# dsilvestro/LiteRate

Measured on AMD Instinct MI355X. Metric: RJMCMC iters/sec x lineages (lineage-log-lik evals/s, summed over chains), higher is better.
Workload: dtype f64

## Files before the change

include/literate_hip.h:

```cpp
#ifndef LITERATE_HIP_H
#define LITERATE_HIP_H

#include <stdint.h>

#ifdef __cplusplus
extern "C" {
#endif

#define LR_OK 0
#define LR_ERR_NULL (-1)
#define LR_ERR_SIZE (-2)
#define LR_ERR_MODEL (-3)
#define LR_ERR_WORKSPACE (-4)
#define LR_ERR_T0 (-5)
#define LR_ERR_STATE (-6)
#define LR_ERR_ORDER (-7)

#define LR_KMAX 32
#define LR_ROW 64
#define LR_MAX_BINS 4094

#define LR_MODEL_BD 0
#define LR_MODEL_ID 1
#define LR_MODEL_KEIDING 2
// ... 177 lines not shown
    int32_t persistent;
    int32_t reserved1;
    int64_t status;
    int64_t xchg;
    int32_t team_blocks;
    int32_t table_mode;
    int64_t lineage_frac;
    int64_t pack_tmp;
    int32_t spec_chains_per_team;
    int32_t streaming;
    int32_t packed_scan;
    int32_t reserved3;
} lr_mcmc_layout;

#define LR_ROW_L 0
#define LR_ROW_M 1
#define LR_ROW_TL 2
#define LR_ROW_TM 3
#define LR_ROW_PL 4
#define LR_ROW_PM 5
#define LR_ROW_PTL 6
#define LR_ROW_PTM 7
#define LR_ROW_SCALARS 8
#define LR_STATE_ROWS 9
#define LR_S_LIKA 0
#define LR_S_PRIORA 1
#define LR_S_PRIORPOIA 2
#define LR_S_GRATE_L 3
#define LR_S_GRATE_M 4
#define LR_S_POI 5
#define LR_S_HASTING 6
#define LR_S_PRIOR_P 7
#define LR_S_PRIORPOI_P 8
#define LR_S_CONST_P 9
#define LR_S_CONST_A 10
#define LR_S_LIK_P 11
#define LR_S_LOG_G0 12
#define LR_S_LOG_G1 13
#define LR_S_LOG_POI 14
#define LR_S_LOG_U 15
#define LR_IROW_EL 0
#define LR_IROW_EM 1
#define LR_IROW_PEL 2
#define LR_IROW_PEM 3
#define LR_IROW_SCALARS 4
#define LR_ISTATE_ROWS 5
#define LR_I_KL 0
#define LR_I_KM 1
#define LR_I_PKL 2
#define LR_I_PKM 3
#define LR_I_GIBBS 4
#define LR_I_INVALID 5
#define LR_I_IT_LO 6
#define LR_I_IT_HI 7
#define LR_I_ACCEPTED 8
#define LR_I_MOVE 9
#define LR_I_NEXT_LO 10
#define LR_I_NEXT_HI 11
#define LR_I_SLOT 12

#define LR_TRACE_HEAD 13
#define LR_TRACE_W (LR_TRACE_HEAD + 2 * (2 * LR_KMAX - 1))

typedef struct lr_engine lr_engine;

int lr_mcmc_query_layout(const lr_mcmc_config* cfg , lr_mcmc_layout* out );
int lr_mcmc_create(const lr_mcmc_config* cfg , const double* ts, const double* te,
                   const double* br_length ,
                   void* workspace, int64_t workspace_bytes, lr_engine** out );
int lr_mcmc_init(lr_engine* e, const double* L, const double* M, const double* tL,
                 const double* tM, const int32_t* KL, const int32_t* KM, int32_t kmax, void* stream);
int lr_mcmc_steps(lr_engine* e, int64_t n_iters, void* stream);
int lr_mcmc_restore(lr_engine* e, void* stream);
int lr_mcmc_time_scan(lr_engine* e, int32_t reps, float* avg_ms , void* stream);
int lr_mcmc_time_steps(lr_engine* e, int64_t n_iters, float* total_ms , void* stream);
int lr_mcmc_status(lr_engine* e, int32_t* status , void* stream);
#define LR_WARN_KCAP 2
int lr_mcmc_warnings(lr_engine* e, int32_t* warnings , void* stream);
int lr_mcmc_describe(const lr_engine* e, char* buf , int32_t n);
int lr_mcmc_p4_config(const lr_engine* e, int32_t* word );
int lr_mcmc_p4_resident(const lr_engine* e, int32_t out[4] );
int lr_mcmc_p4_pipe(const lr_engine* e, int32_t out[4] );
int lr_mcmc_p4_draws(const lr_engine* e, int32_t* out );
int lr_mcmc_destroy(lr_engine* e);

#ifdef __cplusplus
}
#endif
#endif
```

literate_amd/_hip.py:

```python
import ctypes as C
import os

from .build import LIB

c_i32, c_i64, c_f64, c_vp = C.c_int32, C.c_int64, C.c_double, C.c_void_p

LR_ERR_NULL, LR_ERR_SIZE, LR_ERR_MODEL, LR_ERR_WORKSPACE, LR_ERR_T0, LR_ERR_STATE, LR_ERR_ORDER = -1, -2, -3, -4, -5, -6, -7
ERRORS = {-1: "LR_ERR_NULL", -2: "LR_ERR_SIZE", -3: "LR_ERR_MODEL", -4: "LR_ERR_WORKSPACE", -5: "LR_ERR_T0",
          -6: "LR_ERR_STATE", -7: "LR_ERR_ORDER (lineages must be sorted by birth time for the persistent engines)"}

LR_KMAX, LR_ROW, LR_MAX_BINS = 32, 64, 4094
LR_ADE_MAX_BINS = 512
LR_ADEJ_MAX_BINS, LR_ADEJ_MOVES, LR_ADEJ_STATE_W, LR_ADEJ_ROW_W = 128, 5, 96, 73
LR_MLIK_MAX_BINS, LR_MLIK_MAX_TEMPS, LR_MLIK_MOVES, LR_MLIK_STATE_W, LR_MLIK_ROW_W = 512, 128, 2, 16, 12
LR_TMLIK_MAX_BINS, LR_TMLIK_MAX_TEMPS, LR_TMLIK_MAX_MODELS, LR_TMLIK_MOVES, LR_TMLIK_STATE_W, LR_TMLIK_ROW_W = 512, 128, 64, 2, 16, 12
LR_RJBIN_MAX_BINS, LR_RJBIN_STATE_W = 512, 448
LR_RJMC3_MAX_TEMPS, LR_RJMC3_S_POS, LR_RJMC3_LADDER_W, LR_RJMC3_WIDE_MAX_BINS, LR_P_SWAP = 8, 9, 4, 256, 11
LR_WARN_KCAP = 2
LR_STATE_ROWS, LR_ISTATE_ROWS = 9, 5
LR_TRACE_HEAD = 13
LR_TRACE_W = LR_TRACE_HEAD + 2 * (2 * LR_KMAX - 1)
LR_SIMBATCH_GROUPS, LR_SIMBATCH_LDS_SLOTS = 512, 16384
LR_SHIFT_PRIOR_KCAP, LR_SHIFT_PRIOR_BLOCKS = 64, 768
LR_ESS_LDS_ROWS = 16384
# ... 45 lines not shown

SIGNATURES = {
    "lr_version": (c_i32, []),
    "lr_bin_events_workspace_bytes": (c_i64, [c_i64, c_i32]),
    "lr_bin_events": (c_i32, [c_vp, c_vp, c_i64, c_vp, c_vp, c_i32, c_vp, c_vp, c_vp, c_vp, c_i64, c_vp]),
    "lr_bin_unit_events_workspace_bytes": (c_i64, [c_i64, c_i32]),
    "lr_bin_unit_events": (c_i32, [c_vp, c_vp, c_i64, c_f64, c_i32, c_vp, c_vp, c_vp, c_vp, c_i64, c_vp]),
    "lr_expand_rates": (c_i32, [c_vp, c_vp, c_vp, c_i32, c_i32, c_i32, c_i32, c_vp, c_vp]),
    "lr_bd_loglik_workspace_bytes": (c_i64, [c_i64, c_i32, c_i32, c_i32]),
    "lr_bd_loglik_plan": (c_i32, [c_i64, c_i32, c_i32, c_i32, C.POINTER(c_i32)]),
    "lr_bd_loglik_batch": (c_i32, [c_vp, c_vp, c_i64, c_f64, c_i32, c_vp, c_vp, c_i32, c_i32, c_vp, c_f64, c_vp,
                                   c_vp, c_i64, c_vp]),
    "lr_waic_workspace_bytes": (c_i64, [c_i64, c_i32, c_i32, c_i32]),
    "lr_waic_plan": (c_i32, [c_i64, c_i32, c_i32, c_i32, C.POINTER(c_i32)]),
    "lr_waic_pointwise": (c_i32, [c_vp, c_vp, c_i64, c_f64, c_i32, c_vp, c_vp, c_i32, c_i32, c_vp, c_f64, c_vp, c_vp, c_vp,
                                  c_i64, c_vp]),
    "lr_loo_workspace_bytes": (c_i64, [c_i64, c_i32, c_i32, c_i32]),
    "lr_loo_plan": (c_i32, [c_i64, c_i32, c_i32, c_i32, C.POINTER(c_i32)]),
    "lr_loo_pointwise": (c_i32, [c_vp, c_vp, c_i64, c_f64, c_i32, c_vp, c_vp, c_i32, c_i32, c_vp, c_f64, c_vp, c_vp, c_vp,
                                 c_i64, c_vp]),
    "lr_psis_rows_workspace_bytes": (c_i64, [c_i64, c_i32]),
    "lr_psis_rows": (c_i32, [c_vp, c_i64, c_i32, c_vp, c_vp, c_vp, c_i64, c_vp]),
    "lr_rj_propose_score": (c_i32, [c_vp, c_vp, c_vp, c_i32, c_i32, c_vp, c_vp, c_vp, c_f64, c_vp, c_vp, c_vp, c_vp,
                                    c_vp]),
    "lr_log_priors": (c_i32, [c_vp, c_vp, c_i32, c_i32, c_f64, c_vp, c_vp, c_vp, c_vp]),
    "lr_dd_rates": (c_i32, [c_vp, c_vp, c_i32, c_i32, c_i32, c_i32, c_vp, c_vp, c_vp, c_vp, c_vp]),
    "lr_ddv2_rates": (c_i32, [c_vp, c_vp, c_i32, c_i32, c_i32, c_i32, c_vp, c_vp, c_vp, c_vp, c_vp]),
    "lr_binned_keiding": (c_i32, [c_vp, c_vp, c_vp, c_vp, c_vp, c_i32, c_i32, c_vp, c_vp, c_vp]),
    "lr_simulate_bd": (c_i32, [c_vp, c_vp, c_i32, c_i32, c_f64, c_f64, c_f64, c_f64, c_i64, c_i64, C.c_uint64, c_vp, c_vp,
                             c_vp, c_vp, c_vp, c_i64, c_vp]),
    "lr_simulate_bd_batch_workspace_bytes": (c_i64, [c_i32, c_i32, c_i32, c_i64]),
    "lr_simulate_bd_batch": (c_i32, [c_vp, c_vp, c_i32, c_i32, c_i32, c_vp, c_i64, C.c_uint64, c_vp, c_vp, c_vp, c_i64,
                                   c_vp]),
    "lr_simulate_dd_batch_workspace_bytes": (c_i64, [c_i32, c_i32, c_i32, c_i64]),
    "lr_simulate_dd_batch": (c_i32, [c_vp, c_vp, c_i32, c_i32, c_i32, c_i32, c_i32, c_vp, c_i64, C.c_uint64, c_vp, c_vp, c_vp,
                                   c_i64, c_vp]),
    "lr_trend_rates": (c_i32, [c_vp, c_vp, c_i32, c_i32, c_i32, c_i32, c_vp, c_vp, c_vp]),
    "lr_format_rows": (c_i64, [c_vp, c_vp, c_i64, C.c_uint64, c_i32, c_vp, c_i64]),
    "lr_rtt_summary_workspace_bytes": (c_i64, [c_i32, c_i32, c_f64, c_f64, c_f64, c_i32]),
    "lr_rtt_summary": (c_i32, [c_vp, c_i32, c_i32, c_f64, c_f64, c_f64, c_i32, c_vp, c_vp, c_vp, c_vp, c_i64, c_vp]),
    "lr_shift_prior": (c_i32, [c_f64, c_f64, c_i64, c_i64, C.c_uint64, c_f64, c_i32, c_vp, c_vp, c_vp, c_vp, c_vp]),
    "lr_ppc_age_workspace_bytes": (c_i64, [c_i64, c_i32, c_i32]),
    "lr_ppc_age_plan": (c_i32, [c_i64, c_i32, c_i32, C.POINTER(c_i32)]),
    "lr_ppc_age": (c_i32, [c_vp, c_vp, c_i64, c_f64, c_i32, c_vp, c_i32, C.c_uint64, c_vp, c_vp, c_vp, c_vp, c_i64, c_vp]),
    "lr_ade_classes": (c_i32, [c_vp, c_vp, c_i64, c_f64, c_i32, c_vp, c_vp, c_vp, c_vp]),
    "lr_ade_profile_workspace_bytes": (c_i64, [c_i32, c_i32, c_i32]),
    "lr_ade_profile": (c_i32, [c_vp, c_vp, c_i32, c_vp, c_i32, c_vp, c_i32, c_vp, c_vp, c_vp, c_vp, c_i64, c_vp]),
    "lr_adej_workspace_bytes": (c_i64, [c_i32]),
    "lr_adej_prepare": (c_i32, [c_vp, c_vp, c_i32, c_vp, c_i64, c_vp]),
    "lr_adej_loglik": (c_i32, [c_vp, c_i64, c_i32, c_vp, c_vp, c_i32, c_vp, c_vp, c_vp]),
    "lr_adej_init": (c_i32, [c_vp, c_i64, c_i32, c_f64, c_i32, c_i32, c_f64, c_f64, C.c_uint64, c_i32, c_i32, c_vp, c_vp]),
    "lr_adej_steps": (c_i32, [c_vp, c_i64, c_i32, c_f64, c_i32, c_i32, c_f64, c_f64, C.c_uint64, c_i32, c_i32, c_vp, c_i64, c_i64,
                              c_i32, c_vp, c_i64, c_vp]),
    "lr_mlik_init": (c_i32, [c_vp, c_vp, c_vp, c_i32, c_f64, c_f64, c_i32, c_i32, c_f64, c_vp, c_vp, c_i32, C.c_uint64, c_i32, c_i32,
                             c_vp, c_vp]),
    "lr_mlik_steps": (c_i32, [c_vp, c_vp, c_vp, c_i32, c_f64, c_f64, c_i32, c_i32, c_f64, c_vp, c_vp, c_i32, C.c_uint64, c_i32, c_i32,
                              c_vp, c_i64, c_i64, c_i32, c_vp, c_i64, c_vp]),
    "lr_mlik_estimate": (c_i32, [c_vp, c_i64, c_i32, c_i32, c_i64, c_vp, c_vp, c_vp, c_vp, c_vp, c_vp, c_vp, c_vp]),
    "lr_tmlik_init": (c_i32, [C.POINTER(TmlikProblem)]),
    "lr_tmlik_steps": (c_i32, [C.POINTER(TmlikProblem), c_i64, c_i64, c_i32, c_vp, c_i64, c_i64]),
    "lr_rjbin_init": (c_i32, [C.POINTER(RjbinProblem), c_vp, c_vp, c_vp, c_vp, c_vp, c_vp]),
    "lr_rjbin_steps": (c_i32, [C.POINTER(RjbinProblem), c_i64, c_i64, c_i32, c_vp, c_i64, c_i64]),
    "lr_rjmc3_init": (c_i32, [C.POINTER(Rjmc3Problem), c_vp, c_vp, c_vp, c_vp, c_vp, c_vp]),
    "lr_rjmc3_steps": (c_i32, [C.POINTER(Rjmc3Problem), c_i64, c_i64, c_i32, c_vp, c_vp, c_i64, c_i64]),
    "lr_ess_summary_workspace_bytes": (c_i64, [c_i32, c_i32, c_i32, c_vp, c_i32, c_f64, c_i32]),
    "lr_ess_summary": (c_i32, [c_vp, c_i32, c_i32, c_i32, c_vp, c_i32, c_f64, c_i32, c_vp, c_vp, c_vp, c_vp, c_i64, c_vp]),
    "lr_col_summary_workspace_bytes": (c_i64, [c_i32, c_i32, c_i32, c_vp, c_i32, c_f64, c_i32, c_i32]),
    "lr_col_summary": (c_i32, [c_vp, c_i32, c_i32, c_i32, c_vp, c_i32, c_f64, c_i32, c_vp, c_vp, c_i64, c_vp]),
    "lr_curve_summary_workspace_bytes": (c_i64, [c_i32, c_i32, c_i32, c_i32, c_i32, c_i32, c_f64, c_i32, c_i32]),
    "lr_curve_summary": (c_i32, [c_vp, c_i32, c_i32, c_i32, c_i32, c_i32, c_i32, c_i32, c_vp, c_i32, c_f64, c_i32, c_vp,
                                 c_vp, c_i64, c_vp]),
    "lr_mcmc_query_layout": (c_i32, [C.POINTER(McmcConfig), C.POINTER(McmcLayout)]),
    "lr_mcmc_create": (c_i32, [C.POINTER(McmcConfig), c_vp, c_vp, c_vp, c_vp, c_i64, C.POINTER(c_vp)]),
    "lr_mcmc_init": (c_i32, [c_vp, c_vp, c_vp, c_vp, c_vp, c_vp, c_vp, c_i32, c_vp]),
    "lr_mcmc_steps": (c_i32, [c_vp, c_i64, c_vp]),
    "lr_mcmc_time_scan": (c_i32, [c_vp, c_i32, C.POINTER(C.c_float), c_vp]),
    "lr_mcmc_time_steps": (c_i32, [c_vp, c_i64, C.POINTER(C.c_float), c_vp]),
    "lr_mcmc_restore": (c_i32, [c_vp, c_vp]),
    "lr_mcmc_describe": (c_i32, [c_vp, C.c_char_p, c_i32]),
    "lr_mcmc_p4_config": (c_i32, [c_vp, C.POINTER(c_i32)]),
    "lr_mcmc_p4_resident": (c_i32, [c_vp, C.POINTER(c_i32)]),
    "lr_mcmc_p4_pipe": (c_i32, [c_vp, C.POINTER(c_i32)]),
    "lr_mcmc_p4_draws": (c_i32, [c_vp, C.POINTER(c_i32)]),
    "lr_mcmc_status": (c_i32, [c_vp, C.POINTER(c_i32), c_vp]),
    "lr_mcmc_warnings": (c_i32, [c_vp, C.POINTER(c_i32), c_vp]),
    "lr_mcmc_destroy": (c_i32, [c_vp]),
    "lr_debug_draws": (c_i32, [C.c_uint64, c_i64, c_vp, c_vp, c_vp, c_vp, c_vp, c_i32, c_vp, c_vp]),
    "lr_debug_stream2": (c_i32, [c_vp, c_vp, c_i64, c_vp, c_vp]),
}

_lib = None


class HipLibraryError(RuntimeError):
    pass


def load():
    global _lib
    if _lib is not None:
        return _lib
    if not os.path.exists(LIB):
        raise HipLibraryError("libliterate_hip.so not found at %s - run `python -m literate_amd.build` "
                              "(there is no CPU fallback)" % LIB)
    lib = C.CDLL(LIB)
    for name, (res, args) in SIGNATURES.items():
        fn = getattr(lib, name)
        fn.restype, fn.argtypes = res, args
    _lib = lib
    return lib


def check(rc, what):
    if rc == 0:
        return
    if rc < 0:
        raise ValueError("%s: %s" % (what, ERRORS.get(rc, rc)))
    raise HipLibraryError("%s: hipError_t %d" % (what, rc))


def require_gpu():
    import torch
    if not torch.cuda.is_available():
        raise HipLibraryError("no ROCm GPU visible: literate_amd has no CPU path")
    return torch


def ptr(t):
    return None if t is None else c_vp(t.data_ptr())


def stream_ptr(device=None):
    import torch
    return c_vp(torch.cuda.current_stream(device).cuda_stream)


def launch(fn, device, *args):
    import torch
    with torch.cuda.device(device):
        return fn(*args, stream_ptr(device))


def launch_problem(fn, device, problem, *args):
    import torch
    with torch.cuda.device(device):
        problem.stream = stream_ptr(device)
        return fn(C.byref(problem), *args)
```

literate_amd/csrc/lr_engine.h:

```cpp
#pragma once
#include <cmath>
#include "lr_internal.h"
#include "lr_plan.h"
#include "lr_scan.h"
#include "lr_step.h"

struct lr_part {
    int base, count, hA;
    bool pipelined;
    hipStream_t stream;
    hipEvent_t done;
    hipGraphExec_t graph_exec;
    int graph_units;
};

struct lr_p4_shares {
    int delta[16];
    int n_slots;
    int help_trips;
};

struct lr_engine {
    lr_mcmc_config cfg;
    lr_mcmc_layout lay;
    lr_engine_plan plan;
    const double* ts;
    const double* te;
    const double* br_length;
    char* ws;
    bool initialised;
    lr_part part[LR_MAX_PARTS];
    long long n8;
    long long n8_alloc;
    lr_p4_shares p4;
    bool p4_help;
    int p4_cfg;
    bool p4_resident;
    bool p4_pipe;
    bool p4_lean;
    bool packed_scan;
    bool streaming;
    hipEvent_t fork;
    hipEvent_t ev0, ev1;
};


#ifndef LR_SPEC_SCAN_UNROLL
#define LR_SPEC_SCAN_UNROLL 1
#endif
#ifndef LR_SPEC_SCAN_PRIO
#define LR_SPEC_SCAN_PRIO 2
#endif
#define LR_SPEC_TIMEOUT_TICKS 200000000ull

static inline bool lr_p4_help_choice(const lr_engine* e) {
    const char* env = getenv("LR_P4_HELP");
    if (e->lay.persistent != 2 || e->plan.scan.unit == LR_TAB_PAIRGEN || e->cfg.sampler != 0 || e->plan.scan.H > 264) return false;
    return env ? atoi(env) != 0 : true;
}

static inline int lr_p4_cfg_choice(const lr_engine* e) {
    const char* env = getenv("LR_P4_GENERIC");
    if (!lr_p4_help_choice(e) || (env && atoi(env) != 0)) return LR_P4_CFG_GENERIC;
    const lr_mcmc_config& c = e->cfg;
    if (c.const_rates != 0 || c.use_rate_HP == 0 || c.poisson_HP != 0.0) return LR_P4_CFG_GENERIC;
    if (c.frac_birth != LR_P4_FRAC_BIRTH || std::signbit(c.frac_birth) || c.frac_death != LR_P4_FRAC_DEATH) return LR_P4_CFG_GENERIC;
    if (c.model == LR_MODEL_BD || c.model == LR_MODEL_ID) return LR_P4_CFG_BDI;
    return c.model == LR_MODEL_KEIDING ? LR_P4_CFG_KEIDING : LR_P4_CFG_GENERIC;
}

static inline bool lr_p4_resident_choice(const lr_engine* e) {
    const char* env = getenv("LR_P4_RESIDENT");
    return lr_p4_help_choice(e) && !(env && atoi(env) == 0);
}

static inline bool lr_p4_pipe_choice(const lr_engine* e) {
    const char* env = getenv("LR_P4_PIPE");
    return lr_p4_resident_choice(e) && !(env && atoi(env) == 0);
}

static inline bool lr_p4_lean_choice(const lr_engine* e) {
    const char* env = getenv("LR_P4_LEAN_DRAWS");
    return lr_p4_pipe_choice(e) && !(env && atoi(env) == 0);
}

static inline int lr_spec_mode(const lr_engine* e) {
    if (e->lay.spec_chains_per_team != 1) return 0;
    if (e->lay.team_blocks > 1) return 1;
    const double trips = (double)e->n8 / 64.0 / 8.0;
    const char* env = getenv("LR_SPEC_PLANES_BY_SCANNERS");
    const bool by_scanners = env ? atoi(env) != 0 : trips <= 3.0;
    return by_scanners ? 2 : 3;
}

#define LR_STEP_WAVES_PER_BLOCK (LR_SCAN_THREADS / LR_WAVE)
#define LR_STREAM_MAX_CHAINS 16
struct lr_stream_sync {
    unsigned long long arrived;
    unsigned long long pad0[15];
    unsigned long long word[LR_STREAM_COPIES][LR_STREAM_MAX_CHAINS];
};
static_assert(sizeof(lr_stream_sync) + 128 == LR_STREAM_SYNC_BYTES && LR_STREAM_SYNC_BYTES % 256 == 0, "counter line + a line per copy");
int lr_launch_stream(lr_engine* e, const lr_step_args& a, int64_t n_iters, bool query, hipStream_t stream);

int lr_packscan_pairs(const lr_scan_plan& p, int n_chains);
int lr_launch_packscan(const lr_engine* e, int base, int count, hipStream_t stream);

lr_step_args lr_make_args(const lr_engine* e);
int lr_pack_lineages(lr_engine* e, hipStream_t stream);
int lr_launch_spec(lr_engine* e, const lr_step_args& a, const lr_packed_lineages& pk, int64_t n_iters, hipStream_t stream);
```

literate_amd/csrc/lr_mcmc.hip:

```cpp
#include <cmath>
#include <cstdio>
#include <cstdlib>
#include <new>
#include <type_traits>

#include "lr_chain.h"
#include "lr_dd.h"
#include "lr_engine.h"
#include "lr_internal.h"
#include "lr_scan.h"
#include "lr_step.h"

__global__ __launch_bounds__(LR_WAVE) void lr_rj_propose_score_kernel(
    const double* __restrict__ rates, const double* __restrict__ times, const int* __restrict__ K, int kmax,
    const int* __restrict__ move, const int* __restrict__ index, const double* __restrict__ draws, double mult_d,
    double* __restrict__ out_rates, double* __restrict__ out_times, int* __restrict__ out_K,
    double* __restrict__ out_score) {
    const int c = blockIdx.x, lane = threadIdx.x;
    int k = K[c];
    double R = (lane < k) ? rates[(size_t)c * kmax + lane] : 0.0;
    double T = (lane <= k) ? times[(size_t)c * (kmax + 1) + lane] : 0.0;
    const double* dr = draws + (size_t)c * 2 * kmax;
    const int mv = move[c];
    double score = 0.0;
// ... 74 lines not shown

__global__ __launch_bounds__(LR_SCAN_THREADS) void lr_chain_step_kernel(lr_step_args a, int mode, int chain_base,
                                                                        int n_sub) {
    __shared__ lr_seg_scratch scratch[LR_STEP_WAVES];
    const int wave = threadIdx.x / LR_WAVE, lane = threadIdx.x & (LR_WAVE - 1);
    const int j = blockIdx.x * LR_STEP_WAVES + wave;
    if (j < n_sub) lr_chain_step_body<32>(a, mode, chain_base + j, lane, &scratch[wave]);
}

struct lr_fused_args {
    const double* ts;
    const double* te;
    long long n, chunk;
    double t0;
    int n_bins, tiles;
    int scan_base, scan_n;
    int step_base, step_n;
    int step_blocks;
};

template <int CB, int H, bool UNIT>
__global__ __launch_bounds__(LR_SCAN_THREADS) void lr_fused_iter_kernel(lr_step_args a, lr_fused_args f) {
    extern __shared__ double2 lds[];
    lr_seg_scratch* scratch = reinterpret_cast<lr_seg_scratch*>(lds);
    const int bid = blockIdx.x;
    if (bid < f.step_blocks) {
        const int wave = threadIdx.x / LR_WAVE, lane = threadIdx.x & (LR_WAVE - 1);
        const int j = bid * LR_STEP_WAVES + wave;
        if (j < f.step_n) lr_chain_step_body(a, 0, f.step_base + j, lane, &scratch[wave]);
        return;
    }
    int group, tile;
    if ((f.step_blocks & 7) == 0) {
        lr_xcd_remap(bid - f.step_blocks, f.tiles, (f.scan_n + CB - 1) / CB, &group, &tile);
    } else {
        const int sb = bid - f.step_blocks;
        tile = sb % f.tiles, group = sb / f.tiles;
    }
    const double2* tables = a.tables + (size_t)f.scan_base * a.tab_stride;
    const int tile_stride = lr_tile_stride(a.tiles);
    double* partials = const_cast<double*>(a.partials) + (size_t)f.scan_base * tile_stride;
    if (UNIT)
        lr_scan_unit_body<CB, H>(lds, tile, group * CB, f.ts, f.te, f.n, f.t0, f.n_bins, tables, f.scan_n, f.chunk,
                                 partials, tile_stride);
    else
        lr_scan_fast_body<CB, H>(lds, tile, group * CB, f.ts, f.te, f.n, f.t0, f.n_bins, tables, f.scan_n, f.chunk,
                                 partials, tile_stride);
}

#ifndef LR_PERSIST_THREADS
#define LR_PERSIST_THREADS 512
#endif
#ifndef LR_PERSIST_MINWAVES
#define LR_PERSIST_MINWAVES 4
#endif

template <int H, bool GENERAL>
__global__ __launch_bounds__(256) void lr_pairscan_kernel(lr_packed_lineages pk, long long n8, const double2* __restrict__ tables,
                                                          int n_chains, int n_bins, int tiles, double* __restrict__ partials) {
    constexpr int ENT = GENERAL ? 2 : 1;
    __shared__ double2 tab[LR_UNIT_PLANES * H];
    __shared__ double red[4][2];
    const int tid = threadIdx.x, lane = tid & (LR_WAVE - 1), wave = tid / LR_WAVE;
    const int tile = blockIdx.x, pair = blockIdx.y;
    const double2* src = tables + (size_t)pair * (2 * H * ENT);
    for (int i = tid; i < 2 * H * ENT; i += 256) tab[GENERAL ? lr_pairgen_lds_entry(i, H) : i] = src[i];
    __syncthreads();
    if (GENERAL) lr_pair_planes_block_general(tab, H, n_bins, tid, 256);
    else lr_pair_planes_block(tab, H, n_bins, tid, 256);
    __syncthreads();
    const long long per = (n8 + tiles - 1) / tiles;
    const long long g0 = min((long long)tile * per, n8), g1 = min(g0 + per, n8);
    double acc0 = 0.0, acc1 = 0.0;
    lr_persist_scan<H, GENERAL>(reinterpret_cast<const char*>(tab), pk, g0, g1 - g0, tid, 256, &acc0, &acc1);
    const double s0 = lr_wave_sum(acc0), s1 = lr_wave_sum(acc1);
    if (lane == 0) red[wave][0] = s0, red[wave][1] = s1;
    __syncthreads();
    if (tid < 2 && 2 * pair + tid < n_chains)
        partials[(size_t)(2 * pair + tid) * lr_tile_stride(tiles) + tile] = ((red[0][tid] + red[1][tid]) + red[2][tid]) + red[3][tid];
}

typedef __attribute__((address_space(3))) double lr_lds_f64;
typedef __attribute__((address_space(3))) int lr_lds_i32;
template <int PB, int ES, bool PRE = false, int SAMPLER = -1, bool HAND = false, int CFG = LR_P4_CFG_GENERIC, bool LEAN = false>
__device__ __forceinline__ void lr_persist_step_body(const __attribute__((address_space(3))) lr_step_args* a3, int c, int lane,
                                                     __attribute__((address_space(3))) lr_seg_scratch* scratch3,
                                                     lr_lds_f64* st_f64, lr_lds_i32* st_i32, double lik, lr_lds_f64* table3,
                                                     lr_lds_f64* br3 ,
                                                     const lr_draw_slot* draws = nullptr ,
                                                     lr_table_hand* hand = nullptr, int hand_epoch = 0) {
    constexpr int table_es = ES;
    const lr_step_args& a = *(const lr_step_args*)a3;
    const double* br_lds = (const double*)br3;
    LR_SSTAMP(0);
    lr_chain_regs st;
    lr_chain_load(st, (double*)st_f64, (int*)st_i32, lane);
    if (SAMPLER == 1 || (SAMPLER == -1 && a.cfg.sampler != 0))
        lr_dd_step_core<true>(st, a, 0, c, lane, lik, reinterpret_cast<double2*>((double*)table3), table_es, br_lds);
    else if (PRE) {
        lr_rj_draws pre;
        lr_draws_load(draws, pre, lane);
        lr_chain_step_core<true, PB, HAND, CFG, LEAN>(st, a, 0, c, lane, (lr_seg_scratch*)scratch3, lik, reinterpret_cast<double2*>((double*)table3),
                                           table_es, br_lds, br_lds + LR_H_WIDE, &pre, hand, hand_epoch);
    } else
        lr_chain_step_core<true, PB>(st, a, 0, c, lane, (lr_seg_scratch*)scratch3, lik, reinterpret_cast<double2*>((double*)table3),
                                     table_es, br_lds, br_lds + LR_H_WIDE);
    if (HAND) lr_chain_store_handed(st, (double*)st_f64, (int*)st_i32, lane);
    else lr_chain_store(st, (double*)st_f64, (int*)st_i32, lane);
    LR_SSTAMP(8);
}

template <int NA, int BATCH = NA>
__device__ __forceinline__ void lr_p4_leave_sums(double2 (*part)[LR_WAVE], int* arrived, double* out, int slot, int lane,
                                                 int& scans_done, double s0, double s1) {
    part[slot][lane] = make_double2(s0, s1);
    int prev = 0;
    if (lane == 0) prev = __hip_atomic_fetch_add(arrived, 1, __ATOMIC_RELAXED, __HIP_MEMORY_SCOPE_WORKGROUP);
    prev = __builtin_amdgcn_readfirstlane(prev);
    if (prev == NA * (scans_done + 1) - 1) {
        asm volatile("" ::: "memory");
        double a0 = 0.0, a1 = 0.0;
#pragma unroll
        for (int w = 0; w < NA; ++w) {
            if (BATCH < NA && w > 0 && w % BATCH == 0) asm volatile("" : "+v"(a0), "+v"(a1) :: "memory");
            const double2 v = part[w][lane];
            a0 += v.x, a1 += v.y;
        }
        a0 = lr_wave_sum(a0), a1 = lr_wave_sum(a1);
        if (lane == 0) out[0] = a0, out[1] = a1;
    }
    ++scans_done;
}

template <int PB, int ES>
__device__ __attribute__((noinline)) void lr_persist_step(const __attribute__((address_space(3))) lr_step_args* a3, int c, int lane,
                                                          __attribute__((address_space(3))) lr_seg_scratch* scratch3,
                                                          lr_lds_f64* st_f64, lr_lds_i32* st_i32, double lik, lr_lds_f64* table3,
                                                          lr_lds_f64* br3) {
    lr_persist_step_body<PB, ES>(a3, c, lane, scratch3, st_f64, st_i32, lik, table3, br3);
}

template <int PB, int ES, int NW, int SAMPLER, bool HELP, int CFG = LR_P4_CFG_GENERIC, int TAG = 0, bool LEAN = false>
__device__ __attribute__((noinline)) void lr_persist4_steppers(const __attribute__((address_space(3))) lr_step_args* a3, int c0,
                                                               int n_chains, int wave, int lane,
                                                               __attribute__((address_space(3))) lr_seg_scratch* scratch3,
                                                               lr_lds_f64* st_f64, lr_lds_i32* st_i32, lr_lds_f64* red,
                                                               lr_lds_f64* tab, int tab_doubles, lr_lds_f64* br3, long long n_iters,
                                                               const lr_draw_slot* draws ,
                                                               lr_table_hand* hands ) {
    static_assert(!HELP || (ES == 2 && SAMPLER == 0), "helper waves: RJ sampler at unit resolution");
    static_assert(CFG == LR_P4_CFG_GENERIC || HELP, "a configuration word comes with the helper waves");
    for (long long iter = 0; iter < n_iters; ++iter) {
#pragma unroll 1
        for (int ph = 0; ph < 2; ++ph) {
#ifdef LR_DIAG
            const unsigned long long dq0 = wall_clock64();
#endif
            const int c = c0 + 2 * ph + wave;
            if (c < n_chains) {
                double lik = 0.0;
#pragma unroll
                for (int w2 = 2; w2 < (ES == 2  ? 3 : NW); ++w2) lik += red[(ph * NW + w2) * 2 + wave];
                lr_persist_step_body<PB, ES, ES == 2  && SAMPLER == 0, SAMPLER, HELP, CFG, LEAN>(
                    a3, c, lane, scratch3, st_f64 + (2 * ph + wave) * (LR_STATE_ROWS * LR_ROW),
                    st_i32 + (2 * ph + wave) * (LR_ISTATE_ROWS * LR_ROW), lik, tab + ph * tab_doubles + wave, br3,
                    draws + (2 * ph + wave), HELP ? hands + wave : nullptr, (int)((2 * iter + ph + 1) & 0x3fffffff));
            }
#ifdef LR_DIAG
            const unsigned long long dq1 = wall_clock64();
#endif
            __syncthreads();
#ifdef LR_DIAG
            if (lane == 0 && blockIdx.x < 64) {
                atomicAdd(&lr_diag_step[16384 + (blockIdx.x * 16 + wave) * 4 + 0], dq1 - dq0);
                atomicAdd(&lr_diag_step[16384 + (blockIdx.x * 16 + wave) * 4 + 1], wall_clock64() - dq1);
            }
#endif
        }
    }
}

template <int H, int T, int PB>
__device__ __attribute__((noinline)) void lr_persist2_steppers(const __attribute__((address_space(3))) lr_step_args* a3, int c, int wave,
                                                               int lane, __attribute__((address_space(3))) lr_seg_scratch* scratch3,
                                                               lr_lds_f64* st_f64, lr_lds_i32* st_i32, lr_lds_f64* red ,
                                                               lr_lds_f64* tab, lr_lds_f64* br3, const uint4* __restrict__ idx8,
                                                               long long n8w, long long n_iters, int prio_shift, int grp) {
    const int tid = wave * LR_WAVE + lane;
    for (long long iter = 0; iter < n_iters; ++iter) {
        if (prio_shift > 0) {
            if (((wall_clock64() >> prio_shift) + grp) & 1) __builtin_amdgcn_s_setprio(1);
            else __builtin_amdgcn_s_setprio(0);
        }
        double acc0 = 0.0, acc1 = 0.0;
        lr_scan_tail tail;
        lr_persist_scan_pair<H, 1, true>((const char*)(const double*)tab, idx8, n8w, tid, T, &acc0, &acc1, nullptr, &tail);
        const double s0 = lr_wave_sum(acc0), s1 = lr_wave_sum(acc1);
        if (lane == 0) red[wave * 2 + 0] = s0, red[wave * 2 + 1] = s1;
        lr_scan_drain(tail);
        __syncthreads();
        double lik = 0.0;
#pragma unroll
        for (int w2 = 0; w2 < T / LR_WAVE; ++w2) lik += red[w2 * 2 + wave];
        lr_persist_step_body<PB, 2>(a3, c, lane, scratch3, st_f64, st_i32, lik, tab + wave, br3);
        __syncthreads();
    }
}

template <int H, int T>
__global__ __launch_bounds__(T, LR_PERSIST_MINWAVES) void lr_persist_kernel(
    const lr_step_args* __restrict__ ap ,
    const uint4* __restrict__ idx8, long long n8, lr_p4_shares sh, long long n_iters, int prio_shift) {
    const lr_step_args& a = *ap;
    __shared__ double2 tab[LR_UNIT_PLANES * H];
    __shared__ double red[T / LR_WAVE][2];
    __shared__ lr_seg_scratch scratch[2];
    __shared__ double st_f64[2][LR_STATE_ROWS * LR_ROW];
    __shared__ int st_i32[2][LR_ISTATE_ROWS * LR_ROW];
    __shared__ lr_step_args a_lds;
    __shared__ double br_lds[2][LR_H_WIDE];
    const int tid = threadIdx.x, lane = tid & (LR_WAVE - 1), wave = tid / LR_WAVE;
    if (tid < (int)(sizeof(lr_step_args) / 4)) reinterpret_cast<int*>(&a_lds)[tid] = reinterpret_cast<const int*>(ap)[tid];
    for (int b = tid; b < LR_H_WIDE; b += blockDim.x) {
        const bool in = b < ap->cfg.n_bins;
        br_lds[0][b] = (in && ap->br_length) ? ap->br_length[b] : 0.0;
        br_lds[1][b] = in ? ap->log_br[b] : 0.0;
    }
    const int c0 = blockIdx.x * 2;
    const int c = c0 + wave;
    const bool stepper = (wave < 2) && (c < a.cfg.n_chains);
    double2* gpair = lr_chain_table(a, c0);
    if (stepper) {
        const double* S = a.state_f64 + (size_t)c * LR_STATE_ROWS * LR_ROW;
        const int* I = a.state_i32 + (size_t)c * LR_ISTATE_ROWS * LR_ROW;
        for (int r = 0; r < LR_STATE_ROWS; ++r) st_f64[wave][r * LR_ROW + lane] = S[r * LR_ROW + lane];
        for (int r = 0; r < LR_ISTATE_ROWS; ++r) st_i32[wave][r * LR_ROW + lane] = I[r * LR_ROW + lane];
    }
    for (int i = tid; i < 2 * H; i += T) tab[i] = gpair[i];
    __syncthreads();
    lr_pair_planes_block(tab, H, a.cfg.n_bins, tid, T);
    __syncthreads();
    const char* lbase = reinterpret_cast<const char*>(tab);
    const long long n8w = sh.delta[0] != 0 ? ((n8 + T - 1) / T + sh.delta[wave]) * T : n8;
    const int grp = (blockIdx.x >> 8) & 1;
#ifdef LR_DIAG
    unsigned long long d_t0 = 0, d_t1 = 0, d_t2 = 0, d_scan = 0, d_red = 0, d_step = 0;
// ... 8 lines not shown
    } else
#endif
    for (long long iter = 0; iter < n_iters; ++iter) {
        if (prio_shift > 0) {
            if (((wall_clock64() >> prio_shift) + grp) & 1) __builtin_amdgcn_s_setprio(1);
            else __builtin_amdgcn_s_setprio(0);
        }
#ifdef LR_DIAG
        d_t0 = wall_clock64();
#endif
        double acc0 = 0.0, acc1 = 0.0;
        lr_scan_tail tail;
        lr_persist_scan_pair<H, 1, true>(lbase, idx8, n8w, tid, T, &acc0, &acc1, nullptr, &tail);
#ifdef LR_DIAG
        if (lane == 0 && blockIdx.x < 512) atomicAdd(&lr_diag_step[20000 + blockIdx.x * 8 + wave], wall_clock64() - d_t0);
#endif
#ifdef LR_DIAG
        d_t1 = wall_clock64();
#endif
        const double s0 = lr_wave_sum(acc0), s1 = lr_wave_sum(acc1);
        if (lane == 0) red[wave][0] = s0, red[wave][1] = s1;
        lr_scan_drain(tail);
        __syncthreads();
#ifdef LR_DIAG
        d_t2 = wall_clock64();
#endif
        if (stepper) {
            double lik = 0.0;
#pragma unroll
            for (int w2 = 0; w2 < T / LR_WAVE; ++w2) lik += red[w2][wave];
            lr_persist_step<(H <= 264 ? lr_bins_per_lane(H) : 0), 2>(
                (const __attribute__((address_space(3))) lr_step_args*)&a_lds, c, lane,
                (__attribute__((address_space(3))) lr_seg_scratch*)&scratch[wave], (lr_lds_f64*)st_f64[wave],
                (lr_lds_i32*)st_i32[wave], lik, (lr_lds_f64*)(reinterpret_cast<double*>(tab) + wave), (lr_lds_f64*)&br_lds[0][0]);
        }
        __syncthreads();
#ifdef LR_DIAG
        d_scan += d_t1 - d_t0, d_red += d_t2 - d_t1, d_step += wall_clock64() - d_t2;
#endif
    }
#ifdef LR_DIAG
    if (lane == 0 && blockIdx.x < 512) {
        unsigned long long* o = lr_diag_step + 4096 * 12 - 4096 + (blockIdx.x * 8 + wave) % 4096;
        (void)o;
    }
    if (tid == 0 && blockIdx.x < 340) {
        lr_diag_step[blockIdx.x * 12 + 9] = d_scan, lr_diag_step[blockIdx.x * 12 + 10] = d_red;
        lr_diag_step[blockIdx.x * 12 + 11] = d_step;
    }
    if (tid == 0 && blockIdx.x < 1024) lr_diag_step[2048 * 12 + blockIdx.x * 2 + 1] = wall_clock64();
#endif
    if (stepper) {
        double* S = a.state_f64 + (size_t)c * LR_STATE_ROWS * LR_ROW;
        int* I = a.state_i32 + (size_t)c * LR_ISTATE_ROWS * LR_ROW;
        for (int r = 0; r < LR_STATE_ROWS; ++r) S[r * LR_ROW + lane] = st_f64[wave][r * LR_ROW + lane];
        for (int r = 0; r < LR_ISTATE_ROWS; ++r) I[r * LR_ROW + lane] = st_i32[wave][r * LR_ROW + lane];
    }
    for (int i = tid; i < 2 * H; i += T) gpair[i] = tab[i];
}

#ifndef LR_P4_THREADS
#define LR_P4_THREADS 1024
#endif
#ifdef LR_DIAG
#define LR_PSTAMP(k) if (threadIdx.x == 0 && blockIdx.x < 64) lr_diag_step[28672 + blockIdx.x * 8 + (k)] = wall_clock64()
#else
#define LR_PSTAMP(k)
#endif

#ifndef LR_P4_NR
#define LR_P4_NR 8
#endif
#ifndef LR_P4_RES_HDR
#define LR_P4_RES_HDR 0
#endif
#ifndef LR_P4_NR_DRAW
#define LR_P4_NR_DRAW 4
#endif
#define LR_P4_RES_HELP 5
#ifndef LR_P4_PIPE
#define LR_P4_PIPE 1
#endif
template <int H, bool GENERAL, bool PARAM ,
          bool HELP = false, int CFG = LR_P4_CFG_GENERIC, int NR = 0, int PIPE = 0, bool LEAN = false>
__global__ __launch_bounds__(LR_P4_THREADS, LR_P4_THREADS / 256) void lr_persist4_kernel(const lr_step_args* __restrict__ ap ,
                                                                       lr_packed_lineages pk, long long n8,
                                                                       lr_p4_shares sh, long long n_iters, char* carry_all) {
    static_assert(!HELP || (!GENERAL && !PARAM), "helper waves: RJ sampler at unit resolution");
    static_assert(CFG == LR_P4_CFG_GENERIC || (HELP && H <= 264), "a configuration word comes with the helper waves");
    static_assert(NR == 0 || HELP, "resident groups come with the helper waves");
    static_assert(PIPE == 0 || (PIPE == 1 && NR > 0), "the one-block form is one of the resident trips");
    static_assert(!LEAN || PIPE > 0, "the lean draw duty comes with the one-block form");
    const lr_step_args& a = *ap;
    LR_PSTAMP(0);
    constexpr int NW = LR_P4_THREADS / LR_WAVE;
    constexpr int W0 = HELP ? 4 : 2;
    constexpr int NS = NW - W0;
    constexpr int LR_P4_SCANNERS = NS * LR_WAVE;
    constexpr int ENT = GENERAL ? 2 : 1;
    constexpr int ES = GENERAL ? 6 * H : 2;
    __shared__ double2 tab[2][LR_UNIT_PLANES * H];
    __shared__ double red[2][NW][2];
    constexpr bool LAST_SUMS = !GENERAL;
    __shared__ double2 part[LAST_SUMS ? NW - 2 : 1][LR_WAVE];
    __shared__ int arrived;
    __shared__ lr_table_hand hands[2];
    __shared__ lr_seg_scratch scratch[2];
    __shared__ double st_f64[4][LR_STATE_ROWS * LR_ROW];
    __shared__ int st_i32[4][LR_ISTATE_ROWS * LR_ROW];
    __shared__ lr_step_args a_lds;
    __shared__ double br_lds[2][LR_H_WIDE];
    __shared__ lr_draw_slot draws_s[4];
    lr_draw_slot* const draws = draws_s;
    const int tid = threadIdx.x, lane = tid & (LR_WAVE - 1), wave = tid / LR_WAVE;
    if (tid < (int)(sizeof(lr_step_args) / 4)) reinterpret_cast<int*>(&a_lds)[tid] = reinterpret_cast<const int*>(ap)[tid];
    for (int b = tid; b < LR_H_WIDE; b += blockDim.x) {
        const bool in = b < ap->cfg.n_bins;
        br_lds[0][b] = (in && ap->br_length) ? ap->br_length[b] : 0.0;
        br_lds[1][b] = in ? ap->log_br[b] : 0.0;
    }
    constexpr bool draw_ahead = !GENERAL && !PARAM;
    auto draw_duty = [&](int pr) {
        const int q = wave - W0, k = q & 1, ch = 2 * pr + k;
        if (!draw_ahead || q < 0 || q >= (HELP ? 2 : 4) || (int)(blockIdx.x * 4) + ch >= ap->cfg.n_chains) return;
        const int* I = st_i32[ch] + LR_IROW_SCALARS * LR_ROW;
        const unsigned long long it = ((unsigned long long)(unsigned int)I[LR_I_IT_HI] << 32 | (unsigned int)I[LR_I_IT_LO]) + 1ull;
        lr_draw_slot* slot = &draws[ch];
        if (LEAN) lr_spec_draw_lean<CFG>(a_lds, (int)(blockIdx.x * 4) + ch, lane, it, slot, I);
        else if (HELP) lr_spec_draw_both<CFG>(a_lds, (int)(blockIdx.x * 4) + ch, lane, it, slot);
        else lr_spec_draw_part(a_lds, (int)(blockIdx.x * 4) + ch, lane, it, slot, q >> 1);
    };
    auto help_duty = [&](int ph, int epoch) {
        const int k = wave - 2;
        const int ch = 2 * ph + k;
        if ((int)(blockIdx.x * 4) + ch >= ap->cfg.n_chains) return;
        lr_table_hand* hand = &hands[k];
#ifdef LR_DIAG
        const unsigned long long dh0 = wall_clock64();
#endif
        while (__hip_atomic_load(&hand->epoch, __ATOMIC_RELAXED, __HIP_MEMORY_SCOPE_WORKGROUP) != epoch) __builtin_amdgcn_s_sleep(1);
        asm volatile("" ::: "memory");
#ifdef LR_DIAG
        if (lane == 0 && blockIdx.x < 64) atomicAdd(&lr_diag_step[16384 + (blockIdx.x * 16 + wave) * 4 + 2], wall_clock64() - dh0);
#endif
        const lr_seg_scratch* sc = &scratch[k];
        const int eL = lane <= LR_KMAX ? sc->edge[0][lane] : 0, eM = lane <= LR_KMAX ? sc->edge[1][lane] : 0;
        double* tabd = reinterpret_cast<double*>(tab[ph]) + k;
        int model = a_lds.cfg.model;
        if (CFG == LR_P4_CFG_BDI) __builtin_assume((unsigned int)model < 2u);
        if (CFG == LR_P4_CFG_KEIDING) model = LR_MODEL_KEIDING;
        constexpr bool fixed = CFG != LR_P4_CFG_GENERIC;
        const double constP = lr_build_tables_segments<(H <= 264 ? lr_bins_per_lane(H) : 1), 2>(
            sc, eL, eM, hand->KL, hand->KM, br_lds[0], br_lds[1], model, a_lds.cfg.n_bins, a_lds.n_cls, fixed ? H : a_lds.H,
            reinterpret_cast<double2*>(tabd), lane, LR_TAB_UNIT, fixed ? LR_P4_FRAC_BIRTH : a_lds.cfg.frac_birth,
            fixed ? LR_P4_FRAC_DEATH : a_lds.cfg.frac_death, ES, nullptr);
        LR_WAVE_LDS_ORDER();
        lr_pair_planes_wave(tabd, H, a_lds.cfg.n_bins, lane, 0);
        if (lane == 0) st_f64[ch][LR_ROW_SCALARS * LR_ROW + LR_S_CONST_P] = constP;
    };
    if (tid == 0) arrived = 0;
    if (tid < 2) hands[tid].epoch = 0;
    for (int i = tid; i < 2 * NW * 2; i += LR_P4_THREADS) (&red[0][0][0])[i] = 0.0;
    int scans_done = 0;
    constexpr int NA = NS + (HELP ? 2 : 0);
    auto leave_sums = [&](int pr, double s0, double s1) {
        if (LAST_SUMS) {
            lr_p4_leave_sums<NA, (NR > 0 ? NA / 2 : NA)>(part, &arrived, &red[pr][2][0], wave >= W0 ? wave - W0 : NS + wave - 2, lane, scans_done, s0, s1);
        } else {
            s0 = lr_wave_sum(s0), s1 = lr_wave_sum(s1);
            if (lane == 0) red[pr][wave][0] = s0, red[pr][wave][1] = s1;
        }
    };
    const int c0 = blockIdx.x * 4;
    const int C = a.cfg.n_chains;
    if (wave < 4 && c0 + wave < C) {
        const int c = c0 + wave;
        const double* S = a.state_f64 + (size_t)c * LR_STATE_ROWS * LR_ROW;
        const int* I = a.state_i32 + (size_t)c * LR_ISTATE_ROWS * LR_ROW;
        for (int r = 0; r < LR_STATE_ROWS; ++r) st_f64[wave][r * LR_ROW + lane] = S[r * LR_ROW + lane];
        for (int r = 0; r < LR_ISTATE_ROWS; ++r) st_i32[wave][r * LR_ROW + lane] = I[r * LR_ROW + lane];
    }
    double2* g0 = lr_chain_table(a, c0);
    double2* g1 = lr_chain_table(a, c0 + 2);
    for (int i = tid; i < 2 * H * ENT; i += LR_P4_THREADS) {
        const int e = GENERAL ? lr_pairgen_lds_entry(i, H) : i;
        tab[0][e] = g0[i], tab[1][e] = g1[i];
    }
    __syncthreads();
    LR_PSTAMP(1);
    if (GENERAL) {
        lr_pair_planes_block_general(tab[0], H, a.cfg.n_bins, tid, LR_P4_THREADS);
        lr_pair_planes_block_general(tab[1], H, a.cfg.n_bins, tid, LR_P4_THREADS);
    } else {
        lr_pair_planes_block(tab[0], H, a.cfg.n_bins, tid, LR_P4_THREADS);
        lr_pair_planes_block(tab[1], H, a.cfg.n_bins, tid, LR_P4_THREADS);
    }
    __syncthreads();
    LR_PSTAMP(2);
    const bool scanner = wave >= W0;
    const bool helper = HELP && (wave == 2 || wave == 3);
    const int sid = tid - W0 * LR_WAVE;
    const long long nh_ = HELP ? (long long)sh.help_trips * (2 * LR_WAVE) : 0;
    const int k_tot = (int)((n8 - nh_ + LR_P4_SCANNERS - 1) / LR_P4_SCANNERS);
    const int k_mine = k_tot + (scanner ? sh.delta[wave - W0] : 0);
    bool any_shift = false;
#pragma unroll
    for (int q = 0; q < NS; ++q) any_shift |= sh.delta[q] != 0;
    const long long nh = HELP ? (long long)sh.help_trips * (2 * LR_WAVE) : 0;
    const long long n8w = any_shift ? (long long)k_mine * LR_P4_SCANNERS : n8 - nh;
    constexpr bool HDR = LR_P4_RES_HDR != 0;
    lr_resident_groups<(NR > 0 ? NR : 1), HDR> res;
    lr_resident_groups<LR_P4_RES_HELP, HDR> hres;
    constexpr int NRD = NR > 0 ? LR_P4_NR_DRAW : 0;
    lr_resident_groups<(NRD > 0 ? NRD : 1), HDR> dres;
    const bool res_scanner = NR > 0 && scanner && !(draw_ahead && wave - W0 < 2);
    auto help_scan = [&](auto pr_, auto resident_) {
        constexpr int pr = decltype(pr_)::value;
        double s0 = 0.0, s1 = 0.0;
        if (decltype(resident_)::value) {
            const long long done = (long long)hres.trips * (2 * LR_WAVE);
            lr_resident_trips<LR_P4_RES_HELP, HDR, (PIPE > 0)>(reinterpret_cast<const char*>(tab[pr]), hres, s0, s1);
            if (nh > done) lr_persist_scan<H, GENERAL, 1, false, false>(reinterpret_cast<const char*>(tab[pr]), pk, done, nh - done, tid - 2 * LR_WAVE, 2 * LR_WAVE, &s0, &s1);
        } else if (nh > 0) lr_persist_scan<H, GENERAL, 1, false, false>(reinterpret_cast<const char*>(tab[pr]), pk, 0, nh, tid - 2 * LR_WAVE, 2 * LR_WAVE, &s0, &s1);
        leave_sums(pr, s0, s1);
    };
    auto scan_resident = [&](auto pr_, double* s0, double* s1, lr_scan_tail* tail) {
        constexpr int pr = decltype(pr_)::value;
        lr_persist_scan_pair_resident<(PIPE > 0)>(reinterpret_cast<const char*>(tab[pr]), pk.idx8 + nh, n8w, sid, LR_P4_SCANNERS, res, s0, s1, tail);
    };
    static_assert(2 * NW * 8 + 4 <= LR_P4_CARRY_BYTES, "");
    char* carry = carry_all ? carry_all + (size_t)blockIdx.x * LR_P4_CARRY_BYTES : nullptr;
    const bool carried = carry && *reinterpret_cast<const int*>(carry + 2 * NW * 8) == 1;
    auto prologue_draws = [&]() { draw_duty(0); };
    if (carried) {
        if (tid < 2 * NW) (&red[0][0][0])[tid] = reinterpret_cast<const double*>(carry)[tid];
        if (scanner) prologue_draws();
    } else if (scanner) {
        double s0 = 0.0, s1 = 0.0;
        lr_scan_tail tail;
        lr_persist_scan<H, GENERAL, 1, false, true>(reinterpret_cast<const char*>(tab[0]), pk, nh, n8w, sid, LR_P4_SCANNERS, &s0, &s1, nullptr, &tail);
        leave_sums(0, s0, s1);
        lr_scan_drain(tail);
        prologue_draws();
    }
    if (helper && !carried) help_scan(std::integral_constant<int, 0>(), std::false_type());
    __syncthreads();
    LR_PSTAMP(3);
    if (helper) {
        if (NR > 0) lr_resident_load(hres, pk.idx8, nh, tid - 2 * LR_WAVE, 2 * LR_WAVE);
        for (long long iter = 0; iter < n_iters; ++iter) {
#pragma unroll 1
            for (int ph = 0; ph < 2; ++ph) {
#ifdef LR_DIAG
                const unsigned long long dq0 = wall_clock64();
#endif
                if (ph == 0) help_scan(std::integral_constant<int, 1>(), std::integral_constant<bool, (NR > 0)>());
                else help_scan(std::integral_constant<int, 0>(), std::integral_constant<bool, (NR > 0)>());
                help_duty(ph, (int)((2 * iter + ph + 1) & 0x3fffffff));
#ifdef LR_DIAG
                const unsigned long long dq1 = wall_clock64();
#endif
                __syncthreads();
#ifdef LR_DIAG
                if (lane == 0 && blockIdx.x < 64) {
                    atomicAdd(&lr_diag_step[16384 + (blockIdx.x * 16 + wave) * 4 + 0], dq1 - dq0);
                    atomicAdd(&lr_diag_step[16384 + (blockIdx.x * 16 + wave) * 4 + 1], wall_clock64() - dq1);
                }
#endif
            }
        }
    } else if (!scanner)
        lr_persist4_steppers<(H <= 264 ? lr_bins_per_lane(H) : 0), ES, NW, PARAM ? 1 : 0, HELP, CFG, NR + 64 * PIPE, LEAN>(
            (const __attribute__((address_space(3))) lr_step_args*)&a_lds, c0, C, wave, lane,
            (__attribute__((address_space(3))) lr_seg_scratch*)&scratch[wave], (lr_lds_f64*)&st_f64[0][0], (lr_lds_i32*)&st_i32[0][0],
            (lr_lds_f64*)&red[0][0][0], (lr_lds_f64*)reinterpret_cast<double*>(tab[0]), 2 * LR_UNIT_PLANES * H,
            (lr_lds_f64*)&br_lds[0][0], n_iters, &draws[0], &hands[0]);
    else if (res_scanner) {
        if constexpr (NR > 0) {
        lr_resident_load(res, pk.idx8 + nh, n8w, sid, LR_P4_SCANNERS);
        for (long long iter = 0; iter < n_iters; ++iter) {
#pragma unroll
            for (int ph = 0; ph < 2; ++ph) {
#ifdef LR_DIAG
                const unsigned long long dq0 = wall_clock64();
#endif
                {
                    double s0 = 0.0, s1 = 0.0;
                    lr_scan_tail tail;
                    if (ph == 0) scan_resident(std::integral_constant<int, 1>(), &s0, &s1, &tail);
                    else scan_resident(std::integral_constant<int, 0>(), &s0, &s1, &tail);
                    leave_sums(1 - ph, s0, s1);
                    lr_scan_drain(tail);
                }
#ifdef LR_DIAG
                const unsigned long long dq1 = wall_clock64();
#endif
                __syncthreads();
#ifdef LR_DIAG
                if (lane == 0 && blockIdx.x < 64) {
                    atomicAdd(&lr_diag_step[16384 + (blockIdx.x * 16 + wave) * 4 + 0], dq1 - dq0);
                    atomicAdd(&lr_diag_step[16384 + (blockIdx.x * 16 + wave) * 4 + 1], wall_clock64() - dq1);
                }
#endif
            }
        }
        }
    } else {
    if constexpr (NRD > 0) lr_resident_load(dres, pk.idx8 + nh, n8w, sid, LR_P4_SCANNERS);
    for (long long iter = 0; iter < n_iters; ++iter) {
#pragma unroll
        for (int ph = 0; ph < 2; ++ph) {
#ifdef LR_DIAG
            const unsigned long long dq0 = wall_clock64();
#endif
            {
                double s0 = 0.0, s1 = 0.0;
                lr_scan_tail tail;
                if constexpr (NRD > 0) {
                    if (ph == 0) lr_persist_scan_pair_resident<(PIPE > 0)>(reinterpret_cast<const char*>(tab[1]), pk.idx8 + nh, n8w, sid, LR_P4_SCANNERS, dres, &s0, &s1, &tail);
                    else lr_persist_scan_pair_resident<(PIPE > 0)>(reinterpret_cast<const char*>(tab[0]), pk.idx8 + nh, n8w, sid, LR_P4_SCANNERS, dres, &s0, &s1, &tail);
                } else
                lr_persist_scan<H, GENERAL, 1, false, true>(reinterpret_cast<const char*>(tab[1 - ph]), pk, nh, n8w, sid, LR_P4_SCANNERS, &s0, &s1, nullptr, &tail);
                leave_sums(1 - ph, s0, s1);
                lr_scan_drain(tail);
                draw_duty(1 - ph);
            }
#ifdef LR_DIAG
            const unsigned long long dq1 = wall_clock64();
#endif
            __syncthreads();
#ifdef LR_DIAG
            if (lane == 0 && blockIdx.x < 64) {
                atomicAdd(&lr_diag_step[16384 + (blockIdx.x * 16 + wave) * 4 + 0], dq1 - dq0);
                atomicAdd(&lr_diag_step[16384 + (blockIdx.x * 16 + wave) * 4 + 1], wall_clock64() - dq1);
            }
#endif
        }
    }
    }
    LR_PSTAMP(4);
    if (wave < 4 && c0 + wave < C) {
        const int c = c0 + wave;
        double* S = a.state_f64 + (size_t)c * LR_STATE_ROWS * LR_ROW;
        int* I = a.state_i32 + (size_t)c * LR_ISTATE_ROWS * LR_ROW;
        for (int r = 0; r < LR_STATE_ROWS; ++r) S[r * LR_ROW + lane] = st_f64[wave][r * LR_ROW + lane];
        for (int r = 0; r < LR_ISTATE_ROWS; ++r) I[r * LR_ROW + lane] = st_i32[wave][r * LR_ROW + lane];
    }
    for (int i = tid; i < 2 * H * ENT; i += LR_P4_THREADS) {
        const int e = GENERAL ? lr_pairgen_lds_entry(i, H) : i;
        g0[i] = tab[0][e], g1[i] = tab[1][e];
    }
    if (carry) {
        if (tid < 2 * NW) reinterpret_cast<double*>(carry)[tid] = (&red[0][0][0])[tid];
        if (tid == 0) *reinterpret_cast<int*>(carry + 2 * NW * 8) = 1;
    }
// ... 40 lines not shown
        } else {
            const lr_dd_params pp = lr_dd_unpack(A);
            lr_dd_build_tables_wave(pp, a.br_length, cfg.m_birth, cfg.m_death, n_bins, a.H, lr_chain_table(a, c), lane,
                                    a.unit, cfg.frac_birth, cfg.frac_death, lr_tab_es(a.unit, a.H));
        }
        for (int r = 0; r < LR_STATE_ROWS; ++r) S[r * LR_ROW + lane] = 0.0;
        for (int r = 0; r < LR_ISTATE_ROWS; ++r) I[r * LR_ROW + lane] = 0;
        S[LR_ROW_L * LR_ROW + lane] = A, S[LR_ROW_PL * LR_ROW + lane] = A;
        int io = 0;
        if (lane == LR_I_KL || lane == LR_I_PKL || lane == LR_I_KM || lane == LR_I_PKM) io = npar;
        I[LR_IROW_SCALARS * LR_ROW + lane] = io;
        return;
    }
    double L = 0.0, M = 0.0, tL = 0.0, tM = 0.0;
    int KL = 1, KM = 1;
    if (L0) {
        KL = KL0[c], KM = KM0[c];
        if (lane < KL) L = L0[(size_t)c * kmax + lane];
        if (lane < KM) M = M0[(size_t)c * kmax + lane];
        if (lane <= KL) tL = tL0[(size_t)c * (kmax + 1) + lane];
        if (lane <= KM) tM = tM0[(size_t)c * (kmax + 1) + lane];
    } else {
        const double l0 = lr_gamma(rng, 0, LR_P_INIT, 0, 2.0) * 2.0;
        const double m0 = lr_gamma(rng, 0, LR_P_INIT, 64, 2.0) * 2.0;
        if (lane == 0) L = l0, M = m0, tL = tM = cfg.start_time;
        if (lane == 1) tL = tM = cfg.end_time;
    }
    const int eL = lr_wave_edges(tL, 1), eM = lr_wave_edges(tM, 1);
    double logL, logM;
    lr_stage_segments(&scratch, L, M, eL, eM, KL, KM, lane, &logL, &logM);
    const double constA = lr_build_tables_segments(&scratch, eL, eM, KL, KM, a.br_length, a.log_br, cfg.model, n_bins,
                                                   a.n_cls, a.H, lr_chain_table(a, c), lane,
                                                   a.unit, cfg.frac_birth, cfg.frac_death, lr_tab_es(a.unit, a.H));
    S[LR_ROW_L * LR_ROW + lane] = L, S[LR_ROW_M * LR_ROW + lane] = M;
    S[LR_ROW_TL * LR_ROW + lane] = tL, S[LR_ROW_TM * LR_ROW + lane] = tM;
    S[LR_ROW_PL * LR_ROW + lane] = L, S[LR_ROW_PM * LR_ROW + lane] = M;
    S[LR_ROW_PTL * LR_ROW + lane] = tL, S[LR_ROW_PTM * LR_ROW + lane] = tM;
    I[LR_IROW_EL * LR_ROW + lane] = eL, I[LR_IROW_EM * LR_ROW + lane] = eM;
    I[LR_IROW_PEL * LR_ROW + lane] = eL, I[LR_IROW_PEM * LR_ROW + lane] = eM;
    const double poi0 = (cfg.poisson_HP == 0.0) ? 1.0 : cfg.poisson_HP;
    double so = 0.0;
    if (lane == LR_S_GRATE_L || lane == LR_S_GRATE_M) so = 1.0;
    if (lane == LR_S_POI) so = poi0;
    if (lane == LR_S_LOG_POI) so = lr_log(poi0);
    if (lane == LR_S_CONST_A || lane == LR_S_CONST_P) so = constA;
    S[LR_ROW_SCALARS * LR_ROW + lane] = so;
    int io = 0;
    if (lane == LR_I_KL || lane == LR_I_PKL) io = KL;
    if (lane == LR_I_KM || lane == LR_I_PKM) io = KM;
    I[LR_IROW_SCALARS * LR_ROW + lane] = io;
}

extern "C" int lr_mcmc_query_layout(const lr_mcmc_config* cfg, lr_mcmc_layout* out) {
    lr_engine_plan plan;
    return lr_plan_layout(cfg, &plan, out);
}

extern "C" int lr_mcmc_create(const lr_mcmc_config* cfg, const double* ts, const double* te, const double* br_length,
                              void* workspace, int64_t workspace_bytes, lr_engine** out) {
    if (!ts || !te || !workspace || !out) return LR_ERR_NULL;
    lr_engine_plan plan;
    lr_mcmc_layout lay;
    int rc = lr_plan_layout(cfg, &plan, &lay);
    if (rc) return rc;
    if ((cfg->model == LR_MODEL_BD || cfg->model == LR_MODEL_ID || cfg->sampler != 0) && !br_length) return LR_ERR_MODEL;
    if (lay.total_bytes > workspace_bytes) return LR_ERR_WORKSPACE;
    lr_engine* e = new (std::nothrow) lr_engine();
    if (!e) return (int)hipErrorOutOfMemory;
    e->cfg = *cfg;
    e->lay = lay;
    e->plan = plan;
    e->ts = ts, e->te = te, e->br_length = br_length;
    e->ws = (char*)workspace;
    e->initialised = false;
    e->n8 = 0;
    e->n8_alloc = lr_groups_alloc(cfg->n_lineages);
    for (int j = 0; j < 16; ++j) e->p4.delta[j] = 0;
    e->p4.n_slots = 8;
    e->p4_help = lr_p4_help_choice(e);
    e->p4_cfg = lr_p4_cfg_choice(e);
    e->p4_resident = lr_p4_resident_choice(e);
    e->p4_pipe = lr_p4_pipe_choice(e);
    e->p4_lean = lr_p4_lean_choice(e);
    e->streaming = false;
    e->packed_scan = plan.packed_scan;
    e->fork = nullptr;
    e->ev0 = e->ev1 = nullptr;
    for (int p = 0; p < plan.n_parts; ++p) {
        lr_part& q = e->part[p];
        q.base = plan.base[p], q.count = plan.base[p + 1] - plan.base[p], q.hA = plan.hA[p], q.pipelined = plan.pipelined[p];
        q.stream = nullptr, q.done = nullptr, q.graph_exec = nullptr, q.graph_units = 0;
    }
    {
        hipError_t he = hipEventCreate(&e->ev0);
        if (he == hipSuccess) he = hipEventCreate(&e->ev1);
        if (he != hipSuccess) {
            lr_mcmc_destroy(e);
            return (int)he;
        }
    }
    if (plan.family == 0 && plan.n_parts > 1) {
        hipError_t he = hipEventCreateWithFlags(&e->fork, hipEventDisableTiming);
        for (int p = 0; p < plan.n_parts && he == hipSuccess; ++p) {
            he = hipStreamCreateWithFlags(&e->part[p].stream, hipStreamNonBlocking);
            if (he == hipSuccess) he = hipEventCreateWithFlags(&e->part[p].done, hipEventDisableTiming);
        }
        if (he != hipSuccess) {
            lr_mcmc_destroy(e);
            return (int)he;
        }
    }
    if (plan.streaming) {
        const int rcq = lr_launch_stream(e, lr_make_args(e), 0, true, nullptr);
        if (rcq != LR_OK && rcq != LR_ERR_STATE) {
            lr_mcmc_destroy(e);
            return rcq;
        }
        e->streaming = rcq == LR_OK;
    }
    *out = e;
    return LR_OK;
}

lr_step_args lr_make_args(const lr_engine* e) {
    lr_step_args a;
    a.cfg = e->cfg;
    a.state_f64 = (double*)(e->ws + e->lay.state_f64);
    a.state_i32 = (int*)(e->ws + e->lay.state_i32);
    a.log_br = (const double*)(e->ws + e->lay.bin_consts);
    a.dd_consts = a.log_br + e->cfg.n_bins;
    a.log_T = log(e->cfg.end_time - e->cfg.start_time);
    a.mult_l = 2.0 * log(LR_MULT_D);
    a.tables = (double2*)(e->ws + e->lay.tables);
    a.partials = (const double*)(e->ws + e->lay.partials);
    a.trace = (double*)(e->ws + e->lay.trace);
    a.br_length = e->br_length;
    a.tab_stride = e->plan.scan.tab_stride;
    a.n_cls = e->plan.scan.n_cls;
    a.tiles = e->plan.scan.tiles;
    a.H = e->plan.scan.H;
    a.unit = e->plan.scan.unit;
    a.cb = e->plan.scan.cb;
    a.warn = (unsigned int*)(e->ws + e->lay.status) + 1;
    return a;
}

template <int H>
static int lr_launch_pairscan(const lr_engine* e, hipStream_t stream) {
    lr_packed_lineages pk;
    pk.idx8 = (const uint4*)(e->ws + e->lay.lineage_idx), pk.frac = (const uint4*)(e->ws + e->lay.lineage_frac);
    pk.fstride = e->n8_alloc;
    const dim3 grid(e->plan.scan.tiles, (e->cfg.n_chains + 1) / 2);
    if (e->plan.scan.unit == LR_TAB_PAIRGEN)
        hipLaunchKernelGGL((lr_pairscan_kernel<H, true>), grid, dim3(256), 0, stream, pk, e->n8,
                           (const double2*)(e->ws + e->lay.tables), e->cfg.n_chains, e->cfg.n_bins, e->plan.scan.tiles, (double*)(e->ws + e->lay.partials));
    else
        hipLaunchKernelGGL((lr_pairscan_kernel<H, false>), grid, dim3(256), 0, stream, pk, e->n8,
                           (const double2*)(e->ws + e->lay.tables), e->cfg.n_chains, e->cfg.n_bins, e->plan.scan.tiles, (double*)(e->ws + e->lay.partials));
    return (int)hipGetLastError();
}

static int lr_enqueue_scan_range(const lr_engine* e, int base, int count, hipStream_t stream) {
    if (e->packed_scan) return lr_launch_packscan(e, base, count, stream);
    if (e->plan.pair_only) {
        if (base != 0 || count != e->cfg.n_chains) return LR_ERR_STATE;
        switch (e->plan.scan.H) {
// ... 156 lines not shown
        return lr_enqueue_step_range(e, a, 0, q.base, q.count, stream);
    }
    int rc = lr_enqueue_fused(e, a, q.base + q.hA, q.count - q.hA, q.base, q.hA, stream);
    if (rc) return rc;
    return lr_enqueue_fused(e, a, q.base, q.hA, q.base + q.hA, q.count - q.hA, stream);
}

static int lr_run_units(lr_engine* e, const lr_step_args& a, lr_part& q, int64_t units, hipStream_t stream) {
    int64_t done = 0;
    const int G = lr_graph_iters();
    if (G > 0 && units >= G) {
        if (!q.graph_exec) {
            hipStream_t cs = nullptr;
            hipGraph_t graph = nullptr;
            hipError_t he = hipStreamCreateWithFlags(&cs, hipStreamNonBlocking);
            if (he != hipSuccess) return (int)he;
            int rc = LR_OK;
            he = hipStreamBeginCapture(cs, hipStreamCaptureModeThreadLocal);
            if (he == hipSuccess) {
                for (int i = 0; i < G && rc == LR_OK; ++i) rc = lr_enqueue_unit(e, a, q, cs);
                he = hipStreamEndCapture(cs, &graph);
            }
            if (he == hipSuccess && rc == LR_OK) he = hipGraphInstantiate(&q.graph_exec, graph, nullptr, nullptr, 0);
            if (graph) (void)hipGraphDestroy(graph);
            (void)hipStreamDestroy(cs);
            if (rc) return rc;
            if (he != hipSuccess) return (int)he;
            q.graph_units = G;
        }
        while (units - done >= q.graph_units) {
            hipError_t he = hipGraphLaunch(q.graph_exec, stream);
            if (he != hipSuccess) return (int)he;
            done += q.graph_units;
        }
    }
    for (; done < units; ++done) {
        const int rc = lr_enqueue_unit(e, a, q, stream);
        if (rc) return rc;
    }
    return LR_OK;
}

static int lr_run_part(lr_engine* e, const lr_step_args& a, lr_part& q, int64_t n_iters, hipStream_t stream) {
    if (!q.pipelined) return lr_run_units(e, a, q, n_iters, stream);
    int rc = lr_enqueue_fused(e, a, q.base, q.hA, q.base, 0, stream);
    if (rc) return rc;
    rc = lr_run_units(e, a, q, n_iters - 1, stream);
    if (rc) return rc;
    rc = lr_enqueue_fused(e, a, q.base + q.hA, q.count - q.hA, q.base, q.hA, stream);
    if (rc) return rc;
    return lr_enqueue_step_range(e, a, 0, q.base + q.hA, q.count - q.hA, stream);
}

extern "C" int lr_mcmc_steps(lr_engine* e, int64_t n_iters, void* stream_) {
    if (!e) return LR_ERR_NULL;
    if (!e->initialised) return LR_ERR_STATE;
    if (n_iters < 0) return LR_ERR_SIZE;
    if (n_iters == 0) return LR_OK;
    hipStream_t stream = (hipStream_t)stream_;
    const lr_step_args a = lr_make_args(e);
    if (e->plan.family) {
        const uint4* idx8 = (const uint4*)(e->ws + e->lay.lineage_idx);
        const bool general = e->plan.scan.unit == LR_TAB_PAIRGEN;
        lr_packed_lineages pk;
        pk.idx8 = idx8, pk.frac = general ? (const uint4*)(e->ws + e->lay.lineage_frac) : nullptr, pk.fstride = e->n8_alloc;
        if (e->n8 <= 0) return LR_ERR_STATE;
        const lr_step_args* ap = (const lr_step_args*)(e->ws + e->lay.args_blob);
        const int blocks = (e->cfg.n_chains + 1) / 2;
        const bool p4 = e->plan.family == 2;
        const bool param = e->cfg.sampler != 0;
        static const int prio = lr_env_int("LR_PERSIST_PRIO", 12);
        const bool wide = e->plan.threads == 1024;
        if (e->plan.family == 3) return lr_launch_spec(e, a, pk, n_iters, stream);
        for (int64_t done = 0; done < n_iters;) {
            const int64_t n = (n_iters - done > 4096) ? 4096 : n_iters - done;
        static const int carry_env = lr_env_int("LR_P4_CARRY", 1);
        char* p4_carry = (p4 && carry_env) ? e->ws + e->lay.xchg : nullptr;
#define LR_P_LAUNCH(HH)                                                                                                       \
    if (p4) {                                                                                                                 \
        const dim3 g4((e->cfg.n_chains + 3) / 4), b4(LR_P4_THREADS);                                                          \
        if (general && param) hipLaunchKernelGGL((lr_persist4_kernel<HH, true, true>), g4, b4, 0, stream, ap, pk, e->n8, e->p4, (long long)n, p4_carry);   \
        else if (general) hipLaunchKernelGGL((lr_persist4_kernel<HH, true, false>), g4, b4, 0, stream, ap, pk, e->n8, e->p4, (long long)n, p4_carry);      \
        else if (param) hipLaunchKernelGGL((lr_persist4_kernel<HH, false, true>), g4, b4, 0, stream, ap, pk, e->n8, e->p4, (long long)n, p4_carry);        \
        else if (LR_P4_NR > 0 && LR_P4_PIPE > 0 && e->p4_help && e->p4_resident && e->p4_pipe && e->p4_lean && e->p4_cfg == LR_P4_CFG_BDI)    \
            hipLaunchKernelGGL((lr_persist4_kernel<(HH <= 264 ? HH : 264), false, false, true, LR_P4_CFG_BDI, LR_P4_NR, LR_P4_PIPE, true>), g4, b4, 0, stream, ap, pk, e->n8, e->p4, (long long)n, p4_carry); \
        else if (LR_P4_NR > 0 && LR_P4_PIPE > 0 && e->p4_help && e->p4_resident && e->p4_pipe && e->p4_lean && e->p4_cfg == LR_P4_CFG_KEIDING)                                   \
            hipLaunchKernelGGL((lr_persist4_kernel<(HH <= 264 ? HH : 264), false, false, true, LR_P4_CFG_KEIDING, LR_P4_NR, LR_P4_PIPE, true>), g4, b4, 0, stream, ap, pk, e->n8, e->p4, (long long)n, p4_carry); \
        else if (LR_P4_NR > 0 && LR_P4_PIPE > 0 && e->p4_help && e->p4_resident && e->p4_pipe && e->p4_lean)                                                                     \
            hipLaunchKernelGGL((lr_persist4_kernel<(HH <= 264 ? HH : 264), false, false, true, LR_P4_CFG_GENERIC, LR_P4_NR, LR_P4_PIPE, true>), g4, b4, 0, stream, ap, pk, e->n8, e->p4, (long long)n, p4_carry); \
        else if (LR_P4_NR > 0 && LR_P4_PIPE > 0 && e->p4_help && e->p4_resident && e->p4_pipe && e->p4_cfg == LR_P4_CFG_BDI)    \
            hipLaunchKernelGGL((lr_persist4_kernel<(HH <= 264 ? HH : 264), false, false, true, LR_P4_CFG_BDI, LR_P4_NR, LR_P4_PIPE>), g4, b4, 0, stream, ap, pk, e->n8, e->p4, (long long)n, p4_carry); \
        else if (LR_P4_NR > 0 && LR_P4_PIPE > 0 && e->p4_help && e->p4_resident && e->p4_pipe && e->p4_cfg == LR_P4_CFG_KEIDING)                                  \
            hipLaunchKernelGGL((lr_persist4_kernel<(HH <= 264 ? HH : 264), false, false, true, LR_P4_CFG_KEIDING, LR_P4_NR, LR_P4_PIPE>), g4, b4, 0, stream, ap, pk, e->n8, e->p4, (long long)n, p4_carry); \
        else if (LR_P4_NR > 0 && LR_P4_PIPE > 0 && e->p4_help && e->p4_resident && e->p4_pipe)                                                                    \
            hipLaunchKernelGGL((lr_persist4_kernel<(HH <= 264 ? HH : 264), false, false, true, LR_P4_CFG_GENERIC, LR_P4_NR, LR_P4_PIPE>), g4, b4, 0, stream, ap, pk, e->n8, e->p4, (long long)n, p4_carry); \
        else if (LR_P4_NR > 0 && e->p4_help && e->p4_resident && e->p4_cfg == LR_P4_CFG_BDI)    \
            hipLaunchKernelGGL((lr_persist4_kernel<(HH <= 264 ? HH : 264), false, false, true, LR_P4_CFG_BDI, LR_P4_NR>), g4, b4, 0, stream, ap, pk, e->n8, e->p4, (long long)n, p4_carry); \
        else if (LR_P4_NR > 0 && e->p4_help && e->p4_resident && e->p4_cfg == LR_P4_CFG_KEIDING)                                              \
            hipLaunchKernelGGL((lr_persist4_kernel<(HH <= 264 ? HH : 264), false, false, true, LR_P4_CFG_KEIDING, LR_P4_NR>), g4, b4, 0, stream, ap, pk, e->n8, e->p4, (long long)n, p4_carry); \
        else if (LR_P4_NR > 0 && e->p4_help && e->p4_resident)                                                                                \
            hipLaunchKernelGGL((lr_persist4_kernel<(HH <= 264 ? HH : 264), false, false, true, LR_P4_CFG_GENERIC, LR_P4_NR>), g4, b4, 0, stream, ap, pk, e->n8, e->p4, (long long)n, p4_carry); \
        else if (e->p4_help && e->p4_cfg == LR_P4_CFG_BDI)       \
            hipLaunchKernelGGL((lr_persist4_kernel<(HH <= 264 ? HH : 264), false, false, true, LR_P4_CFG_BDI>), g4, b4, 0, stream, ap, pk, e->n8, e->p4, (long long)n, p4_carry); \
        else if (e->p4_help && e->p4_cfg == LR_P4_CFG_KEIDING)                                                                \
            hipLaunchKernelGGL((lr_persist4_kernel<(HH <= 264 ? HH : 264), false, false, true, LR_P4_CFG_KEIDING>), g4, b4, 0, stream, ap, pk, e->n8, e->p4, (long long)n, p4_carry); \
        else if (e->p4_help)                                                                                                  \
            hipLaunchKernelGGL((lr_persist4_kernel<(HH <= 264 ? HH : 264), false, false, true>), g4, b4, 0, stream, ap, pk, e->n8, e->p4, (long long)n, p4_carry); \
        else hipLaunchKernelGGL((lr_persist4_kernel<HH, false, false>), g4, b4, 0, stream, ap, pk, e->n8, e->p4, (long long)n, p4_carry);                  \
    } else if (wide) {                                                                                                        \
        hipLaunchKernelGGL((lr_persist_kernel<HH, 1024>), dim3(blocks), dim3(1024), 0, stream, ap, idx8, e->n8, e->p4, (long long)n, 0); \
    } else {                                                                                                                  \
        hipLaunchKernelGGL((lr_persist_kernel<HH, 512>), dim3(blocks), dim3(512), 0, stream, ap, idx8, e->n8, e->p4, (long long)n, prio); \
    }
            switch (e->plan.scan.H) {
                case 40: LR_P_LAUNCH(40); break;
                case 72: LR_P_LAUNCH(72); break;
                case 136: LR_P_LAUNCH(136); break;
                case 264: LR_P_LAUNCH(264); break;
                default: LR_P_LAUNCH(LR_H_WIDE); break;
            }
#undef LR_P_LAUNCH
            const int rc = (int)hipGetLastError();
            if (rc) return rc;
            done += n;
        }
        return LR_OK;
    }
    if (e->streaming) return lr_launch_stream(e, a, n_iters, false, stream);
    if (e->plan.n_parts == 1) return lr_run_part(e, a, e->part[0], n_iters, stream);
    hipError_t he = hipEventRecord(e->fork, stream);
    if (he != hipSuccess) return (int)he;
    for (int p = 0; p < e->plan.n_parts; ++p) {
        lr_part& q = e->part[p];
        he = hipStreamWaitEvent(q.stream, e->fork, 0);
        if (he != hipSuccess) return (int)he;
        const int rc = lr_run_part(e, a, q, n_iters, q.stream);
        if (rc) return rc;
        he = hipEventRecord(q.done, q.stream);
        if (he != hipSuccess) return (int)he;
        he = hipStreamWaitEvent(stream, q.done, 0);
        if (he != hipSuccess) return (int)he;
    }
    return LR_OK;
}

extern "C" int lr_mcmc_time_steps(lr_engine* e, int64_t n_iters, float* total_ms, void* stream_) {
    if (!e || !total_ms) return LR_ERR_NULL;
    hipStream_t stream = (hipStream_t)stream_;
    int rc = (int)hipEventRecord(e->ev0, stream);
    if (rc == LR_OK) rc = lr_mcmc_steps(e, n_iters, stream_);
    if (rc == LR_OK) rc = (int)hipEventRecord(e->ev1, stream);
    if (rc == LR_OK) rc = (int)hipEventSynchronize(e->ev1);
    float ms = 0.f;
    if (rc == LR_OK) rc = (int)hipEventElapsedTime(&ms, e->ev0, e->ev1);
    *total_ms = ms;
    return rc;
}

extern "C" int lr_mcmc_time_scan(lr_engine* e, int32_t reps, float* avg_ms, void* stream_) {
    if (!e || !avg_ms) return LR_ERR_NULL;
    if (!e->initialised) return LR_ERR_STATE;
    if (reps < 1) return LR_ERR_SIZE;
    hipStream_t stream = (hipStream_t)stream_;
    int rc = lr_enqueue_scan(e, stream);
    if (rc == LR_OK) rc = (int)hipEventRecord(e->ev0, stream);
    for (int i = 0; i < reps && rc == LR_OK; ++i) rc = lr_enqueue_scan(e, stream);
    if (rc == LR_OK) rc = (int)hipEventRecord(e->ev1, stream);
    if (rc == LR_OK) rc = (int)hipEventSynchronize(e->ev1);
    float ms = 0.f;
    if (rc == LR_OK) rc = (int)hipEventElapsedTime(&ms, e->ev0, e->ev1);
    *avg_ms = ms / reps;
    return rc;
}

extern "C" int lr_mcmc_status(lr_engine* e, int32_t* status, void* stream_) {
    if (!e || !status) return LR_ERR_NULL;
    unsigned int v = 0;
    hipError_t he = hipMemcpyAsync(&v, e->ws + e->lay.status, sizeof(v), hipMemcpyDeviceToHost, (hipStream_t)stream_);
    if (he == hipSuccess) he = hipStreamSynchronize((hipStream_t)stream_);
    *status = (int32_t)v;
    return (int)he;
}

extern "C" int lr_mcmc_warnings(lr_engine* e, int32_t* warnings, void* stream_) {
    if (!e || !warnings) return LR_ERR_NULL;
    unsigned int v = 0;
    hipError_t he = hipMemcpyAsync(&v, e->ws + e->lay.status + 4, sizeof(v), hipMemcpyDeviceToHost, (hipStream_t)stream_);
    if (he == hipSuccess) he = hipStreamSynchronize((hipStream_t)stream_);
    *warnings = (int32_t)v;
    return (int)he;
}

extern "C" int lr_mcmc_p4_config(const lr_engine* e, int32_t* word) {
    if (!e || !word) return LR_ERR_NULL;
    *word = (e->plan.family == 2 && e->p4_help) ? e->p4_cfg : LR_P4_CFG_GENERIC;
    return LR_OK;
}

extern "C" int lr_mcmc_p4_resident(const lr_engine* e, int32_t* out) {
    if (!e || !out) return LR_ERR_NULL;
    const bool help = e->plan.family == 2 && e->p4_help;
    const long long h = help ? e->p4.help_trips : 0;
    const long long k_tot = (e->n8 - h * 128 + 767) / 768;
    const bool on = help && e->p4_resident && LR_P4_NR > 0;
    out[0] = on ? (int32_t)(k_tot < LR_P4_NR ? k_tot : LR_P4_NR) : 0;
    out[1] = on ? (int32_t)(h < LR_P4_RES_HELP ? h : LR_P4_RES_HELP) : 0;
    out[2] = (int32_t)e->n8;
    out[3] = (int32_t)h;
    return LR_OK;
}

extern "C" int lr_mcmc_p4_pipe(const lr_engine* e, int32_t* out) {
    if (!e || !out) return LR_ERR_NULL;
    out[0] = out[1] = out[2] = out[3] = 0;
    if (!(e->plan.family == 2 && e->p4_help && e->p4_resident && e->p4_pipe && LR_P4_NR > 0 && LR_P4_PIPE > 0)) return LR_OK;
    const long long h = e->p4.help_trips, n = e->n8 - h * 128;
    out[0] = 1;
    for (int q = 0; q < 12; ++q) {
        const long long mine = 64 * q < n ? (n - 64 * q + 767) / 768 : 0;
        if (q < 2) out[2] += mine >= LR_P4_NR_DRAW;
        else out[1] += mine >= LR_P4_NR;
    }
    out[3] = h >= LR_P4_RES_HELP ? 2 : 0;
    return LR_OK;
}

extern "C" int lr_mcmc_p4_draws(const lr_engine* e, int32_t* out) {
    if (!e || !out) return LR_ERR_NULL;
    *out = (e->plan.family == 2 && e->p4_help && e->p4_resident && e->p4_pipe && e->p4_lean && LR_P4_NR > 0 && LR_P4_PIPE > 0) ? 1 : 0;
    return LR_OK;
}

extern "C" int lr_mcmc_describe(const lr_engine* e, char* buf, int32_t n) {
    if (!e || !buf) return LR_ERR_NULL;
    if (n < 64) return LR_ERR_SIZE;
    if (e->plan.family) {
        const char* gen = e->plan.scan.unit == LR_TAB_PAIRGEN ? "true" : "false";
        if (e->plan.family == 3)
            snprintf(buf, (size_t)n, "lr_spec_kernel<%d, %d, %s, %s, %d>", e->plan.scan.H, e->plan.threads, e->cfg.sampler == 0 ? "true" : "false", gen,
                     lr_spec_mode(e));
        else if (e->plan.family == 2)
            snprintf(buf, (size_t)n, "lr_persist4_kernel<%d, %s, %s, %s>", e->plan.scan.H, gen, e->cfg.sampler != 0 ? "true" : "false",
                     e->p4_help ? "true" : "false");
        else snprintf(buf, (size_t)n, "lr_persist_kernel<%d, %d>", e->plan.scan.H, e->plan.threads);
    } else if (e->packed_scan) {
        snprintf(buf, (size_t)n, "lr_packscan_kernel<%d, %d, %s>", lr_packscan_pairs(e->plan.scan, e->cfg.n_chains), e->plan.scan.H,
                 e->plan.scan.unit == LR_TAB_PAIRGEN ? "true" : "false");
    } else if (e->streaming) {
        snprintf(buf, (size_t)n, "lr_stream_kernel<%d, %d, %s>", e->plan.scan.cb, e->plan.scan.H, e->plan.scan.unit ? "true" : "false");
    } else if (e->part[0].pipelined) {
        snprintf(buf, (size_t)n, "lr_fused_iter_kernel<%d, %d, %s>", e->plan.scan.cb, e->plan.scan.H, e->plan.scan.unit ? "true" : "false");
    } else if (e->plan.scan.fast && !e->plan.scan.unit && e->plan.scan.cb == 16) {
        snprintf(buf, (size_t)n, "lr_scan_wide_kernel<%d>", e->plan.scan.H);
    } else if (e->plan.scan.fast) {
        snprintf(buf, (size_t)n, "%s<%d, %d>", e->plan.scan.unit ? "lr_scan_unit_kernel" : "lr_scan_fast_kernel", e->plan.scan.cb, e->plan.scan.H);
    } else {
        snprintf(buf, (size_t)n, "lr_scan_kernel<%d>", e->plan.scan.cb);
    }
    return LR_OK;
}

extern "C" int lr_mcmc_destroy(lr_engine* e) {
    if (!e) return LR_ERR_NULL;
    for (int p = 0; p < e->plan.n_parts; ++p) {
        lr_part& q = e->part[p];
        if (q.graph_exec) (void)hipGraphExecDestroy(q.graph_exec);
        if (q.done) (void)hipEventDestroy(q.done);
        if (q.stream) (void)hipStreamDestroy(q.stream);
    }
    if (e->fork) (void)hipEventDestroy(e->fork);
    if (e->ev0) (void)hipEventDestroy(e->ev0);
    if (e->ev1) (void)hipEventDestroy(e->ev1);
    delete e;
    return LR_OK;
}

#ifdef LR_DIAG
extern "C" int lr_diag_dump_step(unsigned long long* host_out, int n_words) {
    return (int)hipMemcpyFromSymbol(host_out, HIP_SYMBOL(lr_diag_step), (size_t)n_words * 8);
}
extern "C" int lr_diag_dump_seg(unsigned long long* host_out, int n_words, int reset) {
    int rc = (int)hipMemcpyFromSymbol(host_out, HIP_SYMBOL(lr_diag_seg), (size_t)n_words * 8);
    if (reset) {
        static unsigned long long zeros[64 * 16];
        rc = (int)hipMemcpyToSymbol(HIP_SYMBOL(lr_diag_seg), zeros, sizeof(zeros));
    }
    return rc;
}
#endif
```

literate_amd/csrc/lr_pack.hip:

```cpp
#include <cmath>
#include <cstdio>
#include <cstdlib>
#include <cstring>

#include <rocprim/rocprim.hpp>

#include "lr_engine.h"

__device__ __forceinline__ int lr_birth_index(double s, double t0, int n_bins) {
    return min(max(__double2int_rz(floor(s) - t0), -1), n_bins) + 1;
}
__device__ __forceinline__ int lr_death_index(double e, double t0, int n_bins) {
    return min(max(__double2int_rz(ceil(e) - t0), 0), n_bins + 1);
}

__global__ void lr_pack_runs_kernel(const double* __restrict__ ts, long long n, double t0, int n_bins,
                                    int* __restrict__ start_cand) {
    const long long i = (long long)blockIdx.x * blockDim.x + threadIdx.x;
    if (i >= n) return;
    const int a = lr_birth_index(ts[i], t0, n_bins);
    const int ap = i > 0 ? lr_birth_index(ts[i - 1], t0, n_bins) : -1;
    start_cand[i] = (a != ap) ? (int)i : 0;
}

// ... 50 lines not shown
    flag[i] = (head && slot % LR_SLOTS == 0) ? 1 : 0;
}
__global__ void lr_pack_slots_kernel(const double* __restrict__ ts, const double* __restrict__ te, long long n, double t0,
                                     int n_bins, int H, const int* __restrict__ run_start, const int* __restrict__ stretch_start,
                                     const int* __restrict__ head_incl, const int* __restrict__ group_incl, int permute,
                                     int k_tot, long long share_base, lr_p4_shares sh, unsigned short* __restrict__ out, int extant_block,
                                     double end_time, unsigned int* __restrict__ frac, long long fstride) {
    const long long i = (long long)blockIdx.x * blockDim.x + threadIdx.x;
    if (i >= n) return;
    if (((int)i - stretch_start[i]) & 1) return;
    const int rs = run_start[i];
    const int slot_in_run = head_incl[i] - head_incl[rs];
    const int slot = slot_in_run % LR_SLOTS;
    long long g = group_incl[i] - 1;
    if (permute && g >= share_base) g = share_base + lr_share_permute(g - share_base, k_tot, sh);
    unsigned short* grp = out + g * 8;
    bool x0;
    const int d0 = lr_pack_death_entry(ts, te, i, t0, n_bins, extant_block, end_time, &x0);
    const bool pair = i + 1 < n && stretch_start[i + 1] == stretch_start[i];
    int entry = H + d0;
    if (pair) {
        bool x1;
        const int d1 = lr_pack_death_entry(ts, te, i + 1, t0, n_bins, extant_block, end_time, &x1);
        entry = (2 + (d1 - d0)) * H + d0;
    }
    grp[1 + slot] = (unsigned short)(entry << 4);
    auto fix = [](double f) { return fmin(rint(f * 4294967296.0), 4294967295.0); };
    if (frac) {
        const double s0 = ts[i], e0 = te[i];
        double fe = x0 ? fix(s0 - floor(s0)) : fix(ceil(e0) - e0);
        if (pair) {
            const double e1 = te[i + 1];
            fe = fmin(rint((fe + fix(ceil(e1) - e1)) * 0.5), 4294967295.0);
        }
        frac[((size_t)(slot >> 2) * fstride + g) * 4 + (slot & 3)] = (unsigned int)fe;
    }
    if (slot == 0) {
        const int a = lr_birth_index(ts[i], t0, n_bins);
        int cnt = 0, slots = 0;
        long long k = i;
        while (slots < LR_SLOTS && k < n && run_start[k] == rs) {
            const bool pr = k + 1 < n && stretch_start[k + 1] == stretch_start[k];
            cnt += pr ? 2 : 1, k += pr ? 2 : 1, ++slots;
        }
        grp[0] = (unsigned short)((a << 4) | cnt);
        for (int q = slots; q < LR_SLOTS; ++q) grp[1 + q] = (unsigned short)(H << 4);
        if (frac) {
            double sum = 0.0;
            for (long long m = i; m < k; ++m) {
                const double sm = ts[m];
                sum += fix(sm - floor(sm));
            }
            unsigned int* q = frac + ((size_t)2 * fstride + g) * 4;
            q[0] = (unsigned int)__double2loint(sum), q[1] = (unsigned int)__double2hiint(sum);
        }
    }
}

struct lr_max_op {
    __host__ __device__ int operator()(int a, int b) const { return a > b ? a : b; }
};

static size_t lr_scan_tmp_bytes(long long n) {
    size_t b1 = 0, b2 = 0;
    (void)rocprim::inclusive_scan(nullptr, b1, (const int*)nullptr, (int*)nullptr, (size_t)n, lr_max_op());
    (void)rocprim::inclusive_scan(nullptr, b2, (const int*)nullptr, (int*)nullptr, (size_t)n, rocprim::plus<int>());
    return (b1 > b2 ? b1 : b2) + 256;
}

long long lr_pack_tmp_bytes(long long n) {
    return (long long)(4 * lr_align_up64(n * 4, 256) + (long long)lr_scan_tmp_bytes(n) + 256);
}

static void lr_set_shares(lr_engine* e) {
    static const char* env = getenv("LR_P4_SHARES");
    static const int env2 = lr_env_int("LR_P2_SHARE", 0);
    for (int j = 0; j < 16; ++j) e->p4.delta[j] = 0;
    e->p4.help_trips = 0;
    e->p4_help = lr_p4_help_choice(e);
    e->p4_cfg = lr_p4_cfg_choice(e);
    e->p4_resident = lr_p4_resident_choice(e);
    e->p4_pipe = lr_p4_pipe_choice(e);
    e->p4_lean = lr_p4_lean_choice(e);
    if (e->lay.persistent == 2 && e->p4_help) {
        static const int env_t = lr_env_int("LR_P4_HELP_TRIPS", -1);
        const double t = ((double)e->n8 + 512.0) / 896.0;
        int h = (int)lrint(t - 3.5);
        h = h < 0 ? 0 : (h > 5 ? 5 : h);
        e->p4.help_trips = env_t >= 0 ? env_t : h;
        if (e->p4.help_trips < 0) e->p4.help_trips = 0;
        if ((long long)e->p4.help_trips * 128 > e->n8) e->p4.help_trips = 0;
    }
    if (e->lay.persistent == 0 || e->lay.persistent == 3) {
        e->p4.n_slots = 8;
    } else if (e->lay.persistent == 2) {
        e->p4.n_slots = e->p4_help ? 12 : 14;
        int base[7] = {0, 0, 0, 0, 0, 0, 0};
        if (env && e->p4.n_slots == 14) sscanf(env, "%d,%d,%d,%d,%d,%d,%d", &base[0], &base[1], &base[2], &base[3], &base[4], &base[5], &base[6]);
        const long long behind = e->p4_help ? (long long)e->p4.help_trips * 128 : 0;
        const int per = e->p4.n_slots * 64;
        const int k_tot = (int)((e->n8 - behind + per - 1) / per);
        int sum = 0;
        for (int j = 0; j < 7; ++j) {
            int d = (k_tot >= 6) ? (int)lrint((double)base[j] * k_tot / 14.0) : 0;
            if (d < -(k_tot - 1)) d = -(k_tot - 1);
            if (d > LR_P4_MAX_GIVE) d = LR_P4_MAX_GIVE;
            e->p4.delta[2 * j] = e->p4.delta[2 * j + 1] = d;
            sum += d;
        }
        for (int guard = 0; sum != 0 && guard < 64; ++guard) {
            int pick = 0;
            for (int j = 1; j < 7; ++j)
                if (sum > 0 ? e->p4.delta[2 * j] > e->p4.delta[2 * pick] : e->p4.delta[2 * j] < e->p4.delta[2 * pick]) pick = j;
            const int step = sum > 0 ? -1 : 1;
            e->p4.delta[2 * pick] += step, e->p4.delta[2 * pick + 1] += step;
            sum += step;
        }
        if (sum != 0) for (int j = 0; j < 14; ++j) e->p4.delta[j] = 0;
    } else {
        const bool wide2 = e->plan.threads == 1024;
        e->p4.n_slots = wide2 ? 16 : 8;
        const int k_tot = (int)((e->n8 + e->p4.n_slots * 64 - 1) / (e->p4.n_slots * 64));
        int d = (k_tot >= 12) ? (int)lrint((double)env2 * k_tot / 24.0) : 0;
        if (d > LR_P4_MAX_GIVE) d = LR_P4_MAX_GIVE;
        if (e->p4.n_slots == 8)
            for (int j = 0; j < 4; ++j) e->p4.delta[j] = d, e->p4.delta[4 + j] = -d;
        if (e->p4.n_slots == 16 && k_tot >= 6) {
            static const char* envw = getenv("LR_P2W_SHARES");
            int a = 5, b = 2;
            if (envw) sscanf(envw, "%d,%d", &a, &b);
            int da = (int)lrint((double)a * k_tot / 12.0), db = (int)lrint((double)b * k_tot / 12.0);
            if (da > LR_P4_MAX_GIVE) da = LR_P4_MAX_GIVE;
            if (db > LR_P4_MAX_GIVE) db = LR_P4_MAX_GIVE;
            if (da > k_tot - 1) da = k_tot - 1;
            if (db > k_tot - 1) db = k_tot - 1;
            for (int j = 0; j < 4; ++j) e->p4.delta[j] = da, e->p4.delta[4 + j] = db, e->p4.delta[8 + j] = -db, e->p4.delta[12 + j] = -da;
        }
    }
    const long long stride = (long long)e->p4.n_slots * 64;
    const long long k_tot = (e->n8 + stride - 1) / stride;
    int dmax = 0;
    for (int j = 0; j < 16; ++j) dmax = e->p4.delta[j] > dmax ? e->p4.delta[j] : dmax;
    if ((k_tot + dmax + 1) * stride + (e->p4_help ? (long long)e->p4.help_trips * 128 : 0) > e->n8_alloc)
        for (int j = 0; j < 16; ++j) e->p4.delta[j] = 0;
}

int lr_pack_lineages(lr_engine* e, hipStream_t stream) {
    const long long n = e->cfg.n_lineages;
    if (n >= (1ll << 31)) return LR_ERR_SIZE;
    const bool general = e->plan.scan.unit == LR_TAB_PAIRGEN;
    const int extant_block = e->cfg.model == LR_MODEL_KEIDING_DEAD ? 1 : 0;
    char* tmp = e->ws + e->lay.pack_tmp;
    const long long arr = lr_align_up64(n * 4, 256);
    int* run_start = (int*)tmp;
    int* group_incl = (int*)(tmp + arr);
    int* stretch_start = (int*)(tmp + 2 * arr);
    int* head_incl = (int*)(tmp + 3 * arr);
    char* scan_tmp = tmp + 4 * arr;
    size_t scan_bytes = lr_scan_tmp_bytes(n);
    const dim3 grid((unsigned)((n + 255) / 256)), blk(256);
    hipLaunchKernelGGL(lr_pack_runs_kernel, grid, blk, 0, stream, e->ts, n, e->cfg.t0, e->cfg.n_bins, group_incl);
    hipError_t he = rocprim::inclusive_scan(scan_tmp, scan_bytes, (const int*)group_incl, run_start, (size_t)n, lr_max_op(), stream);
    if (he != hipSuccess) return (int)he;
    {
        hipLaunchKernelGGL(lr_pack_stretch_kernel, grid, blk, 0, stream, e->ts, e->te, n, e->cfg.t0, e->cfg.n_bins,
                           (const int*)run_start, extant_block, e->cfg.end_time, general ? 0 : LR_PAIR_DMAX, group_incl);
// ... 34 lines not shown
```

literate_amd/csrc/lr_step.h:

```cpp
#pragma once
#include "lr_chain.h"
#include "lr_dd.h"
#include "lr_internal.h"
#include "lr_scan.h"

struct lr_step_args {
    lr_mcmc_config cfg;
    double* state_f64;
    int* state_i32;
    const double* log_br;
    double2* tables;
    const double* partials;
    double* trace;
    const double* br_length;
    double log_T;
    double mult_l;
    const double* dd_consts;
    int tab_stride, n_cls, tiles, H, unit, cb;
    unsigned int* warn;
};

#define LR_P4_CFG_GENERIC 0
#define LR_P4_CFG_BDI 1
#define LR_P4_CFG_KEIDING 2
// ... 68 lines not shown
    double cuml = 0.0, cumM = 0.0;
    if (n_cls == 2) cuml = lr_wave_exclusive_scan(sumRl, lane, &totRl);
    if (ext) cumM = lr_wave_exclusive_scan(sumM, lane, &totM);
    const double totL = totR - totM;
    const int x0 = H + n_bins + 2;
    sl = sl0, sm = sm0;
    for (int b = b0; b < b1; ++b) {
        while (sl + 1 < KL && sc->edge[0][sl + 1] <= b) ++sl;
        while (sm + 1 < KM && sc->edge[1][sm + 1] <= b) ++sm;
        const double lam = sc->rate[0][sl], mu = sc->rate[1][sm];
        const double llam = sc->lograte[0][sl], lmu = sc->lograte[1][sm];
        double logB = 0.0, logD = 0.0, R = 0.0;
        if (model >= 2) {
            logB = llam, logD = lmu, R = lam + mu;
        } else if (br_length[b] > 0.0) {
            const double lk = log_br[b];
            logB = (model == 0) ? lk + llam : llam;
            logD = lmu + lk;
            R = (model == 0) ? lam + mu : mu;
        }
        lr_put_S(tabd, unit, es, b + 1, logB + cum, R, fs0);
        lr_put_E(tabd, unit, es, H + b + 1, logD - cum, R, fe0);
        cum += R;
        if (n_cls == 2) {
            tab[2 * H + b + 1] = make_double2(logB + cuml, lam);
            tab[3 * H + b + 1] = make_double2(-cuml, -lam);
            cuml += lam;
        }
        if (ext) {
            lr_put_S(tabd, unit, es, x0 + b + 1, -totL - cumM, -mu, fs0);
            cumM += mu;
        }
    }
    if (lane == 0) {
        lr_put_S(tabd, unit, es, 0, 0.0, 0.0, fs0), lr_put_E(tabd, unit, es, H, 0.0, 0.0, fe0);
        lr_put_S(tabd, unit, es, n_bins + 1, totR, 0.0, fs0), lr_put_E(tabd, unit, es, H + n_bins + 1, -totR, 0.0, fe0);
        if (ext) lr_put_S(tabd, unit, es, x0, -totL, 0.0, fs0), lr_put_S(tabd, unit, es, x0 + n_bins + 1, -totR, 0.0, fs0);
        if (n_cls == 2) {
            tab[2 * H] = make_double2(0.0, 0.0);
            tab[3 * H] = make_double2(0.0, 0.0);
            tab[2 * H + n_bins + 1] = make_double2(totRl, 0.0);
            tab[3 * H + n_bins + 1] = make_double2(-totRl, 0.0);
        }
    }
    return lr_wave_sum(csum);
}

struct lr_seg_cache {
    int packL, packM;
    bool reuse;
};

template <int P>
__device__ __forceinline__ void lr_bin_ranks(const lr_seg_scratch* sc, int eL, int eM, int KL, int KM, int n_bins, int lane,
                                             int (&segL)[P], int (&segM)[P]) {
    const int b0 = lane * P;
    int* marks = const_cast<int*>(sc->marks);
    for (int b = lane; b <= n_bins; b += LR_WAVE) marks[b] = 0;
    LR_WAVE_LDS_ORDER();
    if (lane >= 1 && lane < KL) atomicAdd(&marks[eL], 1);
    if (lane >= 1 && lane < KM) atomicAdd(&marks[eM], 0x10000);
    LR_WAVE_LDS_ORDER();
    int cnt[P], tot = 0;
#pragma unroll
    for (int p = 0; p < P; ++p) {
        cnt[p] = (b0 + p <= n_bins) ? marks[b0 + p] : 0;
        tot += cnt[p];
    }
    int run = lr_wave_exclusive_scan_i32(tot);
#pragma unroll
    for (int p = 0; p < P; ++p) {
        run += cnt[p];
        segL[p] = run & 0xffff, segM[p] = run >> 16;
    }
}
template <int P>
__device__ __forceinline__ void lr_pack_ranks(const int (&segL)[P], const int (&segM)[P], int* packL, int* packM) {
    int pl = 0, pm = 0;
#pragma unroll
    for (int p = 0; p < P; ++p) pl |= segL[p] << (8 * p), pm |= segM[p] << (8 * p);
    *packL = pl, *packM = pm;
}

template <int P, int CS = 2>
__device__ __forceinline__ double lr_build_tables_segments_fast(const lr_seg_scratch* sc, int eL, int eM, int KL,
                                                                int KM, const double* __restrict__ br_length,
                                                                const double* __restrict__ log_br, int model,
                                                                int n_bins, int H, double2* __restrict__ tab,
                                                                int lane, int unit, double fs0, double fe0, int es,
                                                                lr_seg_cache* sg = nullptr) {
    double* tabd = reinterpret_cast<double*>(tab);
    auto put_S = [&](int j, double v, double R) { lr_put_S<CS>(tabd, unit, es, j, v, R, fs0); };
    auto put_E = [&](int j, double v, double R) { lr_put_E<CS>(tabd, unit, es, j, v, R, fe0); };
    const int b0 = lane * P;
#ifdef LR_DIAG
    const int c = blockIdx.x * 2 + ((threadIdx.x >> 7) & 1);
#endif
    LR_SSTAMP(9);
    int segL[P], segM[P];
    double k_b[P], lk_b[P];
#pragma unroll
    for (int p = 0; p < P; ++p) {
        segL[p] = 0, segM[p] = 0;
        const int b = min(b0 + p, n_bins - 1);
        k_b[p] = (model < 2) ? br_length[b] : 1.0;
        lk_b[p] = (model < 2) ? log_br[b] : 0.0;
    }
    if (sg && sg->reuse) {
#pragma unroll
        for (int p = 0; p < P; ++p) segL[p] = (sg->packL >> (8 * p)) & 0xff, segM[p] = (sg->packM >> (8 * p)) & 0xff;
    } else {
        lr_bin_ranks<P>(sc, eL, eM, KL, KM, n_bins, lane, segL, segM);
        if (sg) lr_pack_ranks<P>(segL, segM, &sg->packL, &sg->packM);
    }
    LR_SSTAMP(10);
    double logB[P], logD[P], R[P];
    double sumR = 0.0, csum = 0.0;
#pragma unroll
    for (int p = 0; p < P; ++p) {
        const double lam = sc->rate[0][segL[p]], mu = sc->rate[1][segM[p]];
        const double llam = sc->lograte[0][segL[p]], lmu = sc->lograte[1][segM[p]];
        logB[p] = 0.0, logD[p] = 0.0, R[p] = 0.0;
        if (b0 + p < n_bins) {
            if (model >= 2) {
                logB[p] = llam, logD[p] = lmu, R[p] = lam + mu;
            } else if (k_b[p] > 0.0) {
                logB[p] = (model == 0) ? lk_b[p] + llam : llam;
                logD[p] = lmu + lk_b[p];
                R[p] = (model == 0) ? lam + mu : mu;
                if (model == 1) csum -= lam;
            }
        }
        sumR += R[p];
    }
    LR_SSTAMP(11);
    double totR;
    double cum = lr_wave_exclusive_scan(sumR, lane, &totR);
    LR_SSTAMP(12);
#pragma unroll
    for (int p = 0; p < P; ++p) {
        const int b = b0 + p;
        if (b < n_bins) {
            put_S(b + 1, logB[p] + cum, R[p]);
            put_E(H + b + 1, logD[p] - cum, R[p]);
        }
        cum += R[p];
    }
    if (lane == 0) {
        put_S(0, 0.0, 0.0), put_E(H, 0.0, 0.0);
        put_S(n_bins + 1, totR, 0.0), put_E(H + n_bins + 1, -totR, 0.0);
    }
    if (model == LR_MODEL_KEIDING_DEAD && unit != LR_TAB_GENERAL) {
        double mu_b[P], sumM = 0.0;
#pragma unroll
        for (int p = 0; p < P; ++p) {
            mu_b[p] = (b0 + p < n_bins) ? sc->rate[1][segM[p]] : 0.0;
            sumM += mu_b[p];
        }
        double totM;
        double cumM = lr_wave_exclusive_scan(sumM, lane, &totM);
        const double totL = totR - totM;
        const int x0 = H + n_bins + 2;
#pragma unroll
        for (int p = 0; p < P; ++p) {
            const int b = b0 + p;
            if (b < n_bins) put_S(x0 + b + 1, -totL - cumM, -mu_b[p]);
            cumM += mu_b[p];
        }
        if (lane == 0) put_S(x0, -totL, 0.0), put_S(x0 + n_bins + 1, -totR, 0.0);
    }
    LR_SSTAMP(13);
    return (model == 1) ? lr_wave_sum(csum) : 0.0;
}

template <int PB = 0, int CS = 2>
__device__ __forceinline__ double lr_build_tables_segments(const lr_seg_scratch* sc, int eL, int eM, int KL, int KM,
                                                           const double* __restrict__ br_length,
                                                           const double* __restrict__ log_br, int model, int n_bins,
                                                           int n_cls, int H, double2* __restrict__ tab, int lane,
                                                           int unit, double fs0, double fe0, int es = 2,
                                                           lr_seg_cache* sg = nullptr) {
    static_assert(CS == 2 || PB > 0, "a column of its own is written by the one-pass builder only");
    if (PB > 0)
        return lr_build_tables_segments_fast<(PB > 0 ? PB : 1), CS>(sc, eL, eM, KL, KM, br_length, log_br, model, n_bins, H, tab,
                                                                    lane, unit, fs0, fe0, es, sg);
    if (n_cls == 1 && H <= 264 && n_bins <= LR_WAVE * lr_bins_per_lane(H)) {
        switch (lr_bins_per_lane(H)) {
            case 1: return lr_build_tables_segments_fast<1>(sc, eL, eM, KL, KM, br_length, log_br, model, n_bins, H, tab, lane, unit, fs0, fe0, es, sg);
            case 2: return lr_build_tables_segments_fast<2>(sc, eL, eM, KL, KM, br_length, log_br, model, n_bins, H, tab, lane, unit, fs0, fe0, es, sg);
            default: return lr_build_tables_segments_fast<4>(sc, eL, eM, KL, KM, br_length, log_br, model, n_bins, H, tab, lane, unit, fs0, fe0, es, sg);
        }
    }
    if (sg) sg->reuse = false, sg->packL = sg->packM = -1;
    return lr_build_tables_segments_wave(sc, KL, KM, br_length, log_br, model, n_bins, n_cls, H, tab, lane, unit, fs0,
                                         fe0, es);
}

__device__ __forceinline__ void lr_stage_segments(lr_seg_scratch* sc, double L, double M, int eL, int eM, int KL,
                                                  int KM, int lane, double* logL, double* logM, double extra = 1.0,
                                                  double* log_extra = nullptr) {
    const double Mhi = lr_half_lo(M);
    const bool hi = lane >= 32;
    const int j = lane & 31;
    const bool valid = hi ? (j < KM) : (j < KL);
    const bool free63 = KM < LR_KMAX;
    double x = valid ? (hi ? Mhi : L) : 1.0;
    if (lane == LR_WAVE - 1 && free63) x = extra;
    const double lx = lr_log(x);
    if (log_extra) *log_extra = free63 ? lr_bcast(lx, LR_WAVE - 1) : lr_log(extra);
    sc->rate[hi][j] = x;
    sc->lograte[hi][j] = lx;
    if (lane <= LR_KMAX) sc->edge[0][lane] = eL, sc->edge[1][lane] = eM;
    *logL = lx;
    *logM = lr_half_hi(lx);
    LR_WAVE_LDS_ORDER();
}


struct lr_chain_regs {
    double L, M, tL, tM;
    double pL, pM, ptL, ptM;
// ... 179 lines not shown
        }
        double so = lu;
        so = (lane == 1) ? r_a : so;
        so = (lane == 2) ? lr_bcast(ud.b, 1) : so;
        so = (lane == 3) ? lr_bcast(ud.a, 2) : so;
        so = (lane == 4) ? q_b : so;
        so = (lane == 5) ? lr_bcast(ud.a, 3) : so;
        so = (lane == 6) ? lr_bcast(ud.b, 3) : so;
        so = (lane == 7) ? beta : so;
        if (lane < 8) out->sc[lane] = so;
    }
}

#define LR_UD_LANE 32
static_assert(LR_KMAX <= LR_UD_LANE && LR_UD_LANE + 4 <= LR_WAVE, "one lane per rate below the wave-uniform draws");

__device__ __forceinline__ double lr_wave_multiplier_pre(double& R, int K, bool ff, double x, double m, int lane) {
    const bool active = (lane < K) && ff;
    if (active) R = R * m;
    return lr_wave_sum(active ? x : 0.0);
}

template <int CFG = LR_P4_CFG_GENERIC>
__device__ __forceinline__ void lr_spec_draw_both(const lr_step_args& a, int c, int lane, unsigned long long it, lr_draw_slot* out) {
    const lr_mcmc_config& cfg = a.cfg;
    const lr_stream rng{(uint32_t)cfg.seed, (uint32_t)(cfg.chain_offset + c)};
    const int ul = lane - LR_UD_LANE;
    const uint32_t purpose = (ul < 0) ? LR_P_MULT : ((ul == 0) ? LR_P_ACCEPT : (ul == 1 ? LR_P_MOVE : LR_P_RJ));
    const lr_u2 u = lr_pair(rng, it, purpose, ul < 0 ? (uint32_t)lane : (ul == 3 ? 1u : 0u));
    const double x = a.mult_l * (u.b - .5);
    out->x[lane] = x, out->m[lane] = exp(x), out->da[lane] = u.a;
    const double lu = lr_log(ul == 0 ? u.a : 1.0);
    const double r_a = lr_bcast(u.a, LR_UD_LANE + 1), q_b = lr_bcast(u.b, LR_UD_LANE + 2);
    double beta = 0.0;
    if (!(r_a < 0.8) && r_a < 0.999 && (CFG != LR_P4_CFG_GENERIC || cfg.const_rates == 0) && q_b > 0.5) {
        double ga, gb;
        lr_wave_gamma2(rng, it, LR_P_BETA_A, LR_SHAPE_BETA_RJ, LR_P_BETA_B, LR_SHAPE_BETA_RJ, lane, &ga, &gb);
        beta = ga / (ga + gb);
    }
    double so = lr_bcast(lu, LR_UD_LANE);
    so = (lane == 1) ? r_a : so;
    so = (lane == 2) ? lr_bcast(u.b, LR_UD_LANE + 1) : so;
    so = (lane == 3) ? lr_bcast(u.a, LR_UD_LANE + 2) : so;
    so = (lane == 4) ? q_b : so;
    so = (lane == 5) ? lr_bcast(u.a, LR_UD_LANE + 3) : so;
    so = (lane == 6) ? lr_bcast(u.b, LR_UD_LANE + 3) : so;
    so = (lane == 7) ? beta : so;
    if (lane < 8) out->sc[lane] = so;
}

template <int CFG = LR_P4_CFG_GENERIC>
__device__ __forceinline__ void lr_spec_draw_lean(const lr_step_args& a, int c, int lane, unsigned long long it, lr_draw_slot* out,
                                                  const int* I) {
    const lr_mcmc_config& cfg = a.cfg;
    const lr_stream rng{(uint32_t)cfg.seed, (uint32_t)(cfg.chain_offset + c)};
    const int ul = lane - LR_UD_LANE;
    const uint32_t purpose = (ul < 0) ? LR_P_MULT : ((ul == 0) ? LR_P_ACCEPT : (ul == 1 ? LR_P_MOVE : LR_P_RJ));
    const lr_u2 u = lr_pair(rng, it, purpose, ul < 0 ? (uint32_t)lane : (ul == 3 ? 1u : 0u));
    const double r_a = lr_bcast(u.a, LR_UD_LANE + 1), r_b = lr_bcast(u.b, LR_UD_LANE + 1), q_b = lr_bcast(u.b, LR_UD_LANE + 2);
    const unsigned int one = (unsigned int)__ballot(I[lane] == 1);
    const double b_freq = cfg.const_death_rate ? 0.7 : 0.4;
    const bool one_rate = (one & (r_a < b_freq ? (1u << LR_I_KL | 1u << LR_I_PKL) : (1u << LR_I_KM | 1u << LR_I_PKM))) != 0u;
    if (r_a < 0.8 && (r_b < .5 || one_rate)) {
        const double x = a.mult_l * (u.b - .5);
        out->x[lane] = x, out->m[lane] = exp(x), out->da[lane] = u.a;
    }
    double beta = 0.0;
    if (!(r_a < 0.8) && r_a < 0.999 && (CFG != LR_P4_CFG_GENERIC || cfg.const_rates == 0) && q_b > 0.5) {
        double ga, gb;
        lr_wave_gamma2(rng, it, LR_P_BETA_A, LR_SHAPE_BETA_RJ, LR_P_BETA_B, LR_SHAPE_BETA_RJ, lane, &ga, &gb);
        beta = ga / (ga + gb);
    }
    if (ul >= 0 && ul < 4) out->sc[max(2 * ul - 1, 0)] = u.a;
    if (ul >= 1 && ul < 4) out->sc[2 * ul] = u.b;
    if (lane == 7) out->sc[7] = beta;
}

struct lr_table_hand {
    int epoch;
    int KL, KM;
    int reuse;
    int noop;
    int out_idx, base_idx;
    int pad_;
    double par[8];
};

template <bool LDS_CONSTS = false, int PB = 0, int CS = 2, bool PAIR_PLANES = true, bool HAND = false, int CFG = LR_P4_CFG_GENERIC,
          bool LEAN = false>
__device__ __forceinline__ void lr_propose_rj(const lr_step_args& a, int c, int lane, lr_seg_scratch* scratch_p,
                                              uint64_t it, lr_rj_state& s, lr_rj_prop& p, double2* table,
                                              int table_es, const lr_rj_draws* pre = nullptr,
                                              const double* br_lds = nullptr, const double* logbr_lds = nullptr,
                                              const double* base_col = nullptr, int col_doubles = 0, double base_const = 0.0,
                                              lr_table_hand* hand = nullptr, int hand_epoch = 0) {
    static_assert(CS == 2 || (PB > 0 && !PAIR_PLANES), "a column of its own: one-pass builder, no pair planes");
    static_assert(!HAND || PB > 0, "a helper wave runs the one-pass builder");
    static_assert(CFG == LR_P4_CFG_GENERIC || HAND, "a configuration word comes with the helper waves");
    static_assert(!LEAN || HAND, "the lean draw duty is one of the helper-wave form");
    lr_seg_scratch& scratch = *scratch_p;
    const lr_mcmc_config& cfg = a.cfg;
    constexpr bool fixed = CFG != LR_P4_CFG_GENERIC;
    const int n_bins = cfg.n_bins;
    const lr_stream rng{(uint32_t)cfg.seed, (uint32_t)(cfg.chain_offset + c)};
    const double L = s.L, M = s.M, tL = s.tL, tM = s.tM;
    const int eL = s.eL, eM = s.eM, KL = s.KL, KM = s.KM;
    double g0 = s.g0, g1 = s.g1, poi = s.poi, lg0 = s.lg0, lg1 = s.lg1, lpoi = s.lpoi;
    const double priorPoiA = s.priorPoi;

    lr_u2 ud{0.0, 0.0};
    if (!pre) {
        const int ul = lane - LR_UD_LANE;
        const uint32_t purpose = (ul < 0) ? LR_P_MULT : ((ul == 0) ? LR_P_ACCEPT : (ul == 1 ? LR_P_MOVE : LR_P_RJ));
        ud = lr_pair(rng, it, purpose, ul < 0 ? (uint32_t)lane : (ul == 3 ? 1u : 0u));
    }
    const double u_next = pre ? (LEAN ? pre->log_u : 1.0) : lr_bcast(ud.a, LR_UD_LANE);
    LR_SSTAMP(2);

    double pL = L, pM = M, ptL = tL, ptM = tM;
    int peL = eL, peM = eM, PKL = KL, PKM = KM;
    double hasting = 0.0, priorPoi = 0.0;
    int gibbs = 0, invalid = 0, move_kind;
    const double sample_shift_mu = cfg.const_death_rate ? 0.0 : 0.5;
    const double b_freq = cfg.const_death_rate ? 0.7 : 0.4, d_freq = 0.8;
    const double fL = cfg.update_fraction, fM = cfg.const_death_rate ? 1.0 : cfg.update_fraction;
    const lr_u2 r = pre ? lr_u2{pre->r_a, pre->r_b} : lr_u2{lr_bcast(ud.a, LR_UD_LANE + 1), lr_bcast(ud.b, LR_UD_LANE + 1)};
    if (r.a < b_freq) {
        if (r.b < .5 || KL == 1) {
            if (pre) {
                hasting = lr_wave_multiplier_pre(pL, KL, pre->da < fL, pre->x, pre->m, lane);
            } else {
                hasting = lr_wave_multiplier(pL, KL, ud.a < fL, ud.b, a.mult_l, lane);
            }
            move_kind = 0;
        } else {
            peL = lr_wave_edges(tL, 0);
            move_kind = 1;
        }
    } else if (r.a < d_freq) {
        if (r.b < .5 || KM == 1) {
            if (pre) {
                hasting = lr_wave_multiplier_pre(pM, KM, pre->da < fM, pre->x, pre->m, lane);
            } else {
                hasting = lr_wave_multiplier(pM, KM, ud.a < fM, ud.b, a.mult_l, lane);
            }
            move_kind = 2;
        } else {
            peM = lr_wave_edges(tM, 0);
            move_kind = 3;
        }
    } else if (r.a < 0.999 && (fixed || cfg.const_rates == 0)) {
        move_kind = 4;
        const lr_u2 q = pre ? lr_u2{pre->q_a, pre->q_b} : lr_u2{lr_bcast(ud.a, LR_UD_LANE + 2), lr_bcast(ud.b, LR_UD_LANE + 2)};
        const bool sideL = q.a > sample_shift_mu;
        double R = sideL ? L : M, T = sideL ? tL : tM;
        int K = sideL ? KL : KM;
        double score = 0.0;
        const lr_u2 q2 = pre ? lr_u2{pre->q2_a, pre->q2_b} : lr_u2{lr_bcast(ud.a, LR_UD_LANE + 3), lr_bcast(ud.b, LR_UD_LANE + 3)};
        if (q.b > 0.5) {
            if (K >= LR_KMAX) {
                invalid = LR_INVALID_KCAP;
            } else {
                const int ind = min((int)(q2.a * K), K - 1);
                const double delta = q2.b * (lr_bcast(T, ind + 1) - lr_bcast(T, ind));
                double beta;
                if (pre) {
                    beta = pre->beta;
                } else {
                    double ga, gb;
                    lr_wave_gamma2(rng, it, LR_P_BETA_A, LR_SHAPE_BETA_RJ, LR_P_BETA_B, LR_SHAPE_BETA_RJ, lane, &ga, &gb);
                    beta = ga / (ga + gb);
                }
                score = lr_wave_add_shift(R, T, K, ind, delta, beta, lane);
            }
        } else if (K > 1) {
            const int idx = 1 + min((int)(q2.a * (K - 1)), K - 2);
            score = lr_wave_remove_shift(R, T, K, idx, lane);
        }
        hasting = score;
        const int E = lr_wave_edges(T, 0);
        if (sideL) pL = R, ptL = T, PKL = K, peL = E;
        else pM = R, ptM = T, PKM = K, peM = E;
        priorPoi = lr_poisson_prior(PKL, poi, lpoi) + lr_poisson_prior(PKM, poi, lpoi);
    } else {
        move_kind = 5;
        double gl = 0.0, gm = 0.0, gp = 0.0, dummy;
        if (fixed || cfg.use_rate_HP)
            lr_wave_gamma2(rng, it, LR_P_GIBBS_L, LR_HP_GAMMA_SHAPE + LR_GAMMA_SHAPE * KL, LR_P_GIBBS_M,
                           LR_HP_GAMMA_SHAPE + LR_GAMMA_SHAPE * KM, lane, &gl, &gm);
        if (fixed || cfg.poisson_HP == 0.0)
            lr_wave_gamma2(rng, it, LR_P_GIBBS_POI, LR_RJHP_SHAPE + KL + KM, LR_P_GIBBS_POI, LR_RJHP_SHAPE + KL + KM, lane,
                           &gp, &dummy);
        if (fixed || cfg.poisson_HP == 0.0) poi = gp * (1. / (LR_RJHP_RATE + 2));
        if (fixed || cfg.use_rate_HP) {
            const double sL = lr_wave_sum(lane < KL ? L : 0.0), sM = lr_wave_sum(lane < KM ? M : 0.0);
            g0 = gl * (1. / (LR_HP_GAMMA_RATE + sL));
            g1 = gm * (1. / (LR_HP_GAMMA_RATE + sM));
        }
        const double lx = lr_log(lane == 0 ? g0 : (lane == 1 ? g1 : (lane == 2 ? poi : 1.0)));
        lg0 = lr_bcast(lx, 0), lg1 = lr_bcast(lx, 1), lpoi = lr_bcast(lx, 2);
        gibbs = 1;
    }

    LR_SSTAMP(3);
    double logpL, logpM, log_u_next;
    lr_stage_segments(&scratch, pL, pM, peL, peM, PKL, PKM, lane, &logpL, &logpM, u_next, &log_u_next);
    if (pre && !LEAN) log_u_next = pre->log_u;

    lr_seg_cache sg{s.sgL, s.sgM, false};
    bool edges_same = false;
    if ((pre && s.sg_valid) || base_col) edges_same = PKL == KL && PKM == KM && __ballot(lane <= LR_KMAX && (peL != eL || peM != eM)) == 0ull;
    if (pre && s.sg_valid) sg.reuse = edges_same;
    const bool same_table = base_col && edges_same && (move_kind == 1 || move_kind == 3 || move_kind == 5);
    if (HAND) {
        if (lane == 0) hand->KL = PKL, hand->KM = PKM, hand->reuse = sg.reuse ? 1 : 0, hand->noop = same_table ? 1 : 0;
        LR_WAVE_LDS_ORDER();
        if (lane == 0) __hip_atomic_store(&hand->epoch, hand_epoch, __ATOMIC_RELAXED, __HIP_MEMORY_SCOPE_WORKGROUP);
    }

    LR_SSTAMP(4);
    double priorP = -INFINITY;
    {
        const double nL = lr_dpp_zero<0x130 , 0xf, 0xf>(ptL);
        const double nM = lr_dpp_zero<0x130, 0xf, 0xf>(ptM);
        const double dmin = fmin(lane < PKL ? fabs(nL - ptL) : 1e300, lane < PKM ? fabs(nM - ptM) : 1e300);
        if (__ballot(dmin <= LR_MIN_ALLOWED_T)) invalid |= LR_INVALID_GUARD;
    }
    if (!invalid) {
        const double vL = (lane < PKL) ? (logpL + lg0) - pL * g0 + lg0 : 0.0;
        const double vM = (lane < PKM) ? (logpM + lg1) - pM * g1 + lg1 : 0.0;
        priorP = lr_wave_sum(vL + vM);
        priorP += -a.log_T * (PKL - 1 + PKM - 1);
        if (priorPoi != 0.0) priorP += priorPoi;
        else priorP += priorPoiA, priorPoi = priorPoiA;
    }

    LR_SSTAMP(5);
    double constP = 0.0;
    p.table_by_helper = 0;
    if (same_table) {
        double* col = reinterpret_cast<double*>(table);
        for (int i = lane; i < col_doubles; i += LR_WAVE) col[CS * i] = base_col[CS * i];
        constP = base_const;
    } else if (HAND) {
        p.table_by_helper = 1;
    } else {
        constP = lr_build_tables_segments<PB, CS>(&scratch, peL, peM, PKL, PKM, LDS_CONSTS ? br_lds : a.br_length,
                                                  LDS_CONSTS ? logbr_lds : a.log_br, cfg.model,
                                                  n_bins, a.n_cls, a.H, table, lane,
                                                  lr_tab_mode<LDS_CONSTS>(a, table_es), cfg.frac_birth, cfg.frac_death,
                                                  table_es, pre ? &sg : nullptr);
        s.sgL = sg.packL, s.sgM = sg.packM, s.sg_valid = (pre && sg.packL != -1) ? 1 : 0;
    }
    if (LDS_CONSTS && PAIR_PLANES && !HAND && !same_table) {
        LR_WAVE_LDS_ORDER();
        if (lr_tab_mode<LDS_CONSTS>(a, table_es) == LR_TAB_UNIT) lr_pair_planes_wave(reinterpret_cast<double*>(table), a.H, n_bins, lane, 0);
        else lr_pair_planes_wave_general(reinterpret_cast<double*>(table), a.H, n_bins, lane, 0);
    }
    LR_SSTAMP(6);
    s.L = pL, s.M = pM, s.tL = ptL, s.tM = ptM, s.eL = peL, s.eM = peM, s.KL = PKL, s.KM = PKM;
    s.g0 = g0, s.g1 = g1, s.poi = poi, s.lg0 = lg0, s.lg1 = lg1, s.lpoi = lpoi, s.priorPoi = priorPoi;
    p.hasting = hasting, p.prior = priorP, p.constP = constP, p.log_u = log_u_next;
    p.gibbs = gibbs, p.invalid = invalid, p.move = move_kind;
}

template <bool LDS_CONSTS = false, int PB = 0, bool HAND = false, int CFG = LR_P4_CFG_GENERIC, bool LEAN = false>
__device__ __forceinline__ void lr_chain_step_core(lr_chain_regs& st, const lr_step_args& a, int mode, int c, int lane,
                                                   lr_seg_scratch* scratch_p, double lik_sum, double2* table,
                                                   int table_es = 2, const double* br_lds = nullptr,
                                                   const double* logbr_lds = nullptr, const lr_rj_draws* pre = nullptr,
                                                   lr_table_hand* hand = nullptr, int hand_epoch = 0) {
    const lr_mcmc_config& cfg = a.cfg;
    const double sc = st.sc;
    const int isc = st.isc;
    double lik_p = lr_bcast(sc, LR_S_LIK_P);
    double likA = lr_bcast(sc, LR_S_LIKA), priorA = lr_bcast(sc, LR_S_PRIORA);
    double constA = lr_bcast(sc, LR_S_CONST_A);
    lr_rj_state s;
    s.L = st.L, s.M = st.M, s.tL = st.tL, s.tM = st.tM, s.eL = st.eL, s.eM = st.eM;
    s.KL = lr_bcast_i(isc, LR_I_KL), s.KM = lr_bcast_i(isc, LR_I_KM);
    s.g0 = lr_bcast(sc, LR_S_GRATE_L), s.g1 = lr_bcast(sc, LR_S_GRATE_M), s.poi = lr_bcast(sc, LR_S_POI);
    s.lg0 = lr_bcast(sc, LR_S_LOG_G0), s.lg1 = lr_bcast(sc, LR_S_LOG_G1), s.lpoi = lr_bcast(sc, LR_S_LOG_POI);
    s.priorPoi = lr_bcast(sc, LR_S_PRIORPOIA);
    s.sgL = s.sgM = 0, s.sg_valid = 0;
    uint64_t it = (uint64_t)(uint32_t)lr_bcast_i(isc, LR_I_IT_LO) | ((uint64_t)(uint32_t)lr_bcast_i(isc, LR_I_IT_HI) << 32);
    int n_acc = lr_bcast_i(isc, LR_I_ACCEPTED);
    uint64_t next_sample = (uint64_t)(uint32_t)lr_bcast_i(isc, LR_I_NEXT_LO) | ((uint64_t)(uint32_t)lr_bcast_i(isc, LR_I_NEXT_HI) << 32);
    int trace_slot = lr_bcast_i(isc, LR_I_SLOT);
    LR_SSTAMP(1);

    if (mode == 1) {
        likA = lik_sum + constA;
        priorA = lr_wave_prior_gamma(s.L, s.KL, LR_GAMMA_SHAPE, 2.0, lane) + lr_wave_prior_gamma(s.M, s.KM, LR_GAMMA_SHAPE, 2.0, lane);
        priorA += -a.log_T * (s.KL - 1 + s.KM - 1);
        s.priorPoi = lr_poisson_prior(s.KL, s.poi, s.lpoi) + lr_poisson_prior(s.KM, s.poi, s.lpoi);
        priorA += s.priorPoi;
    } else {
        const int gibbs = lr_bcast_i(isc, LR_I_GIBBS), invalid = lr_bcast_i(isc, LR_I_INVALID);
        const double priorP = lr_bcast(sc, LR_S_PRIOR_P), constP = lr_bcast(sc, LR_S_CONST_P);
        double lik;
        const bool ok = lr_mh_accept(gibbs, invalid, lik_sum, constP, likA, priorP, priorA, lr_bcast(sc, LR_S_HASTING),
                                     lr_bcast(sc, LR_S_LOG_U), &lik) && mode != 2;
        lik_p = invalid ? -INFINITY : lik;
        lr_warn_kcap(a.warn, invalid, lane);
        if (ok) {
            s.L = st.pL, s.M = st.pM, s.tL = st.ptL, s.tM = st.ptM, s.eL = st.peL, s.eM = st.peM;
            s.KL = lr_bcast_i(isc, LR_I_PKL), s.KM = lr_bcast_i(isc, LR_I_PKM);
            likA = lik, priorA = priorP, s.priorPoi = lr_bcast(sc, LR_S_PRIORPOI_P), constA = constP;
            n_acc += 1;
        }
        if (it == next_sample) {
            const int slot = trace_slot;
            trace_slot += 1;
            next_sample += (uint64_t)cfg.s_freq;
            if (slot < cfg.n_trace_slots) lr_write_trace_row(a, c, lane, slot, it, likA, priorA, s);
        }
        it += 1;
    }
    const double priorPoiA = s.priorPoi;
    st.L = s.L, st.M = s.M, st.tL = s.tL, st.tM = s.tM, st.eL = s.eL, st.eM = s.eM;
    const int KL = s.KL, KM = s.KM;

    lr_rj_prop p;
    if (HAND) lr_propose_rj<LDS_CONSTS, (PB > 0 ? PB : 1), 2, true, HAND, CFG, LEAN>(a, c, lane, scratch_p, it, s, p, table, table_es, pre, br_lds, logbr_lds, nullptr, 0, 0.0, hand, hand_epoch);
    else lr_propose_rj<LDS_CONSTS, PB>(a, c, lane, scratch_p, it, s, p, table, table_es, pre, br_lds, logbr_lds);

    st.pL = s.L, st.pM = s.M, st.ptL = s.tL, st.ptM = s.tM, st.peL = s.eL, st.peM = s.eM;
    {
        double so = 0.0;
        so = (lane == LR_S_LIKA) ? likA : so;
        so = (lane == LR_S_PRIORA) ? priorA : so;
        so = (lane == LR_S_PRIORPOIA) ? priorPoiA : so;
        so = (lane == LR_S_GRATE_L) ? s.g0 : so;
        so = (lane == LR_S_GRATE_M) ? s.g1 : so;
        so = (lane == LR_S_POI) ? s.poi : so;
        so = (lane == LR_S_HASTING) ? p.hasting : so;
        so = (lane == LR_S_PRIOR_P) ? p.prior : so;
        so = (lane == LR_S_PRIORPOI_P) ? s.priorPoi : so;
        so = (lane == LR_S_CONST_P) ? p.constP : so;
        so = (lane == LR_S_CONST_A) ? constA : so;
        so = (lane == LR_S_LIK_P) ? lik_p : so;
        so = (lane == LR_S_LOG_G0) ? s.lg0 : so;
        so = (lane == LR_S_LOG_G1) ? s.lg1 : so;
        so = (lane == LR_S_LOG_POI) ? s.lpoi : so;
        so = (lane == LR_S_LOG_U) ? p.log_u : so;
        st.sc = so;
        int io = 0;
        io = (lane == LR_I_KL) ? KL : io;
        io = (lane == LR_I_KM) ? KM : io;
        io = (lane == LR_I_PKL) ? s.KL : io;
        io = (lane == LR_I_PKM) ? s.KM : io;
        io = (lane == LR_I_GIBBS) ? p.gibbs : io;
        io = (lane == LR_I_INVALID) ? p.invalid : io;
        io = (lane == LR_I_IT_LO) ? (int)(uint32_t)it : io;
        io = (lane == LR_I_IT_HI) ? (int)(uint32_t)(it >> 32) : io;
        io = (lane == LR_I_ACCEPTED) ? n_acc : io;
        io = (lane == LR_I_MOVE) ? p.move : io;
        io = (lane == LR_I_NEXT_LO) ? (int)(uint32_t)next_sample : io;
        io = (lane == LR_I_NEXT_HI) ? (int)(uint32_t)(next_sample >> 32) : io;
        io = (lane == LR_I_SLOT) ? trace_slot : io;
        st.isc = io;
    }
    LR_SSTAMP(7);

}


struct lr_dd_prop {
    double hasting, prior, log_u;
    int move;
};
struct lr_dd_draws {
    double log_u, rr_a, rr_b, slide_u, z1;
    double da, x, m;
};
__device__ __forceinline__ void lr_make_dd_draws(const lr_step_args& a, int c, int lane, uint64_t it, lr_dd_draws& d) {
    const lr_mcmc_config& cfg = a.cfg;
    const bool trend = cfg.sampler == 2;
    const lr_stream rng{(uint32_t)cfg.seed, (uint32_t)(cfg.chain_offset + c)};
    const uint32_t purpose = trend ? (lane == 0 ? LR_P_TR_ACCEPT : LR_P_TR_MOVE)
                                   : (lane == 0 ? LR_P_DD_ACCEPT : (lane == 1 ? LR_P_DD_MOVE : LR_P_DD_SLIDE));
    const lr_u2 ud = lr_pair(rng, it, purpose, 0u);
    const double lu = lr_log(lane == 0 ? ud.a : 1.0);
    d.log_u = lr_bcast(lu, 0);
    d.rr_a = lr_bcast(ud.a, 1), d.rr_b = lr_bcast(ud.b, 1), d.slide_u = lr_bcast(ud.a, 2);
    d.z1 = 0.0, d.da = 1.0, d.x = 0.0, d.m = 1.0;
    if (trend) {
        const lr_u2 u = lr_pair(rng, it, LR_P_TR_MULT, lane);
        d.da = u.a;
        if (d.rr_a < .33) {
            d.x = lr_normal(rng, it, LR_P_TR_NORM, lane);
        } else {
            d.x = a.mult_l * (u.b - .5);
            d.m = exp(d.x);
        }
    } else if (d.rr_b < 0.1 && (cfg.m_birth == 2 || cfg.m_death == 2)) {
        if (cfg.m_death == -1) d.z1 = lr_normal(rng, it, LR_P_DD_SLIDE, 1);
    } else {
        const lr_u2 u = lr_pair(rng, it, LR_P_DD_MULT, lane);
        d.da = u.a;
        d.x = a.mult_l * (u.b - .5);
        d.m = exp(d.x);
    }
}

template <bool LDS_CONSTS, bool PAIR_PLANES, int CS>
__device__ __forceinline__ void lr_param_tables(const lr_step_args& a, double P, const double* aux, double2* table, int mode,
// ... 216 lines not shown
```

literate_amd/engine.py:

```python
import ctypes as C
import hashlib
import os
from collections import namedtuple

import numpy as np

from . import _hip, ops


class ChainEngine:
    def __init__(self, ts, te, n_chains, model=0, seed=1, const_rates=0, const_death_rate=0, use_rate_HP=1,
                 poisson_HP=0.0, update_fraction=0.75, s_freq=1000, n_trace_slots=0, chain_offset=0,
                 device=None, stats=None, sort_lineages=True, unit_resolution=None, engine="auto", dd=None, team=0,
                 chains_per_team=0):
        torch = _hip.require_gpu()
        self.lib = _hip.load()
        self.device = torch.device(device or "cuda")
        ts_d = ops._dev(ts, torch.float64, self.device)
        te_d = ops._dev(te, torch.float64, self.device)
        if sort_lineages:
            o1 = torch.sort(te_d, stable=True).indices
            o2 = torch.sort(torch.floor(ts_d[o1]), stable=True).indices
            order = o1[o2]
            ts_d, te_d = ts_d[order].contiguous(), te_d[order].contiguous()
# ... 129 lines not shown
            self._init_keep = [ops._dev(args, torch.float64, self.device)]
            rc = _hip.launch(self.lib.lr_mcmc_init, self.device, self.handle, _hip.ptr(self._init_keep[0]), None, None, None,
                             None, None, _hip.LR_KMAX)
        else:
            kmax = _hip.LR_KMAX
            Ls = np.zeros((self.n_chains, kmax)); Ms = np.zeros((self.n_chains, kmax))
            tLs = np.zeros((self.n_chains, kmax + 1)); tMs = np.zeros((self.n_chains, kmax + 1))
            KL = np.zeros(self.n_chains, dtype=np.int32); KM = np.zeros(self.n_chains, dtype=np.int32)
            for c in range(self.n_chains):
                l, m = np.atleast_1d(L[c]), np.atleast_1d(M[c])
                KL[c], KM[c] = len(l), len(m)
                Ls[c, :len(l)], Ms[c, :len(m)] = l, m
                tLs[c, :len(l) + 1], tMs[c, :len(m) + 1] = tL[c], tM[c]
            dev = [ops._dev(x, torch.float64, self.device) for x in (Ls, Ms, tLs, tMs)]
            dk = [ops._dev(x, torch.int32, self.device) for x in (KL, KM)]
            self._init_keep = dev + dk
            rc = _hip.launch(self.lib.lr_mcmc_init, self.device, self.handle, *[_hip.ptr(x) for x in dev + dk], kmax)
        _hip.check(rc, "lr_mcmc_init")
        self.iterations = 0

    def _launch(self, fn, *args):
        import torch
        idx = self.device.index
        if idx is None or torch.cuda.current_device() == idx:
            return fn(*args, C.c_void_p(torch.cuda.current_stream().cuda_stream))
        return _hip.launch(fn, self.device, *args)

    def steps(self, n):
        _hip.check(self._launch(self.lib.lr_mcmc_steps, self.handle, int(n)), "lr_mcmc_steps")
        self.iterations += int(n)

    def time_scan(self, reps=20):
        ms = C.c_float(0.0)
        _hip.check(_hip.launch(self.lib.lr_mcmc_time_scan, self.device, self.handle, int(reps), C.byref(ms)),
                   "lr_mcmc_time_scan")
        return float(ms.value)

    def check_status(self):
        st = C.c_int32(0)
        _hip.check(_hip.launch(self.lib.lr_mcmc_status, self.device, self.handle, C.byref(st)), "lr_mcmc_status")
        if st.value != 0:
            raise _hip.HipLibraryError("engine status %d: a wait between blocks timed out (the kernel's blocks were not all "
                                       "resident: is the GPU shared? LR_SHARED_DEVICE=1 runs without teams, LR_STREAM=0 "
                                       "without the resident streaming kernel), the run is void" % st.value)

    def warnings(self):
        w = C.c_int32(0)
        _hip.check(_hip.launch(self.lib.lr_mcmc_warnings, self.device, self.handle, C.byref(w)), "lr_mcmc_warnings")
        return int(w.value)

    def warning_text(self):
        w = self.warnings()
        if w & _hip.LR_WARN_KCAP:
            return ("WARNING: an add-shift move was proposed from a state with %d rates and rejected: the device holds at "
                    "most %d rates per process (the reference has no cap, LiteRateForward.py:29-47); the posterior of "
                    "the number of shifts is truncated there" % (_hip.LR_KMAX, _hip.LR_KMAX))
        return ""

    def kernel_name(self):
        buf = C.create_string_buffer(128)
        _hip.check(self.lib.lr_mcmc_describe(self.handle, buf, 128), "lr_mcmc_describe")
        return buf.value.decode()

    def p4_config(self):
        w = C.c_int32(0)
        _hip.check(self.lib.lr_mcmc_p4_config(self.handle, C.byref(w)), "lr_mcmc_p4_config")
        return int(w.value)

    def p4_resident(self):
        out = (C.c_int32 * 4)()
        _hip.check(self.lib.lr_mcmc_p4_resident(self.handle, out), "lr_mcmc_p4_resident")
        return tuple(int(v) for v in out)

    def p4_pipe(self):
        out = (C.c_int32 * 4)()
        _hip.check(self.lib.lr_mcmc_p4_pipe(self.handle, out), "lr_mcmc_p4_pipe")
        return tuple(int(v) for v in out)

    def p4_draws(self):
        w = C.c_int32(0)
        _hip.check(self.lib.lr_mcmc_p4_draws(self.handle, C.byref(w)), "lr_mcmc_p4_draws")
        return "lean" if w.value else "full"

    def timed_steps(self, n):
        ms = C.c_float(0.0)
        _hip.check(self._launch(self.lib.lr_mcmc_time_steps, self.handle, int(n), C.byref(ms)), "lr_mcmc_time_steps")
        self.iterations += int(n)
        return float(ms.value)

    def prepared_timed_steps(self, n):
        import torch
        ms = C.c_float(0.0)
        fn, handle, n_c, ms_ref = self.lib.lr_mcmc_time_steps, self.handle, C.c_int64(int(n)), C.byref(ms)
        with torch.cuda.device(self.device):
            stream = C.c_void_p(torch.cuda.current_stream(self.device).cuda_stream)

        def call():
            rc = fn(handle, n_c, ms_ref, stream)
            if rc:
                _hip.check(rc, "lr_mcmc_time_steps")
            self.iterations += int(n)
            return float(ms.value)
        return call

    _CFG_KEYS = ("n_lineages", "n_bins", "n_chains", "model", "const_rates", "const_death_rate", "use_rate_HP",
                 "s_freq", "n_trace_slots", "poisson_HP", "update_fraction", "t0", "start_time", "end_time", "seed",
                 "chain_offset", "unit_resolution", "frac_birth", "frac_death", "sampler", "m_birth", "m_death",
                 "dd_present", "dd_init_death", "engine_mode")

    def _signature(self):
        sig = {k: repr(getattr(self.cfg, k)) for k in self._CFG_KEYS}
        sig.update({"layout_" + f: repr(getattr(self.layout, f)) for f, _ in self.layout._fields_})
        sig["data_sha1"] = self._data_hash
        sig["format"] = "2: state in .npz (head, tail), trace rows in .npz.trace"
        return sig

    def _trace_span(self):
        return int(self.layout.trace), int(self.layout.status)

    def checkpoint_begin(self):
        import torch
        t0, t1 = self._trace_span()
        with torch.cuda.device(self.device):
            head, tail = self.workspace[:t0].clone(), self.workspace[t1:].clone()
            ev = torch.cuda.Event()
            ev.record()
        return dict(head=head, tail=tail, ev=ev, iterations=int(self.iterations), samples=int(self.samples_done()))

    def checkpoint_write(self, ticket, path):
        import torch
        path = str(path)
        if not path.endswith(".npz"):
            path += ".npz"
        side = getattr(self, "_ckpt_stream", None)
        if side is None:
            side = self._ckpt_stream = torch.cuda.Stream(device=self.device)
        row_bytes = self.n_chains * _hip.LR_TRACE_W * 8
        s1 = ticket["samples"]
        sidecar = path + ".trace"
        saved = getattr(self, "_ckpt_saved", {}).get(path, 0)
        if saved > s1 or not os.path.exists(sidecar) or os.path.getsize(sidecar) < saved * row_bytes:
            saved = 0
        with torch.cuda.device(self.device), torch.cuda.stream(side):
            side.wait_event(ticket["ev"])
            head, tail = ticket["head"].cpu().numpy(), ticket["tail"].cpu().numpy()
            new_rows = self.trace[saved:s1].cpu().numpy() if s1 > saved else None
        side.synchronize()
        sig = self._signature()
        tmp = path + ".tmp.npz"
        np.savez(tmp, head=head, tail=tail, iterations=np.int64(ticket["iterations"]), n_trace_rows=np.int64(s1),
                 sig_keys=np.array(list(sig.keys())), sig_vals=np.array(list(sig.values())))
        if saved > 0:
            with open(sidecar, "r+b") as f:
                f.seek(saved * row_bytes)
                f.truncate()
                if new_rows is not None:
                    f.write(new_rows.tobytes())
                f.flush()
                os.fsync(f.fileno())
        else:
            with open(sidecar + ".tmp", "wb") as f:
                if new_rows is not None:
                    f.write(new_rows.tobytes())
                f.flush()
                os.fsync(f.fileno())
            os.replace(sidecar + ".tmp", sidecar)
# ... 171 lines not shown
```

scratch/diag_p4_waves.py:

```python
import sys, os, ctypes
sys.path.insert(0, os.path.dirname(os.path.dirname(os.path.abspath(__file__))))
import torch, numpy as np
from literate_amd import synth, _hip
from literate_amd.engine import ChainEngine
ts, te, _ = synth.make_lineages(100000, 128, 20, 0)
eng = ChainEngine(ts, te, 1024, model=0, seed=1, s_freq=100, n_trace_slots=40, engine="persistent4")
eng.init(); eng.steps(3000); torch.cuda.synchronize()
lib = _hip.load()
N = 16384 + 64 * 16 * 4
buf = (ctypes.c_ulonglong * N)()
lib.lr_diag_dump_step.argtypes = [ctypes.c_void_p, ctypes.c_int]
lib.lr_diag_dump_step(buf, N)
b0 = np.frombuffer(buf, dtype=np.uint64).astype(np.float64)[16384:].reshape(64, 16, 4).copy()
n = 2000
ms = eng.timed_steps(n); torch.cuda.synchronize()
lib.lr_diag_dump_step(buf, N)
b1 = np.frombuffer(buf, dtype=np.uint64).astype(np.float64)[16384:].reshape(64, 16, 4)
d = (b1 - b0) / (2 * n) / 100.0
print("launch: %.2f us per iteration (%.2f per phase)" % (ms * 1e3 / n, ms * 1e3 / n / 2))
print("wave: work / wait (us per phase, mean over 64 blocks)")
for w in range(16):
    help_ = eng.kernel_name().endswith("true>")
    role = "step" if w < 2 else ("help" if help_ and w < 4 else "scan")
    print("  w%-2d %s  %.2f / %.2f%s" % (w, role, d[:, w, 0].mean(), d[:, w, 1].mean(),
                                       "   (of the work: %.2f waiting for the hand-over)" % d[:, w, 2].mean() if role == "help" else ""))
```

Baseline: 17440 billion.

## Split stepper-to-helper table hand-over into two stages to overlap log computation

Adds an EARLY template path in which the stepper wave publishes the proposed rates, edges and segment counts to the helper wave before computing their logs, then signals a second epoch once the log-rates are written. The helper's table builder runs the rate/scan part of the build right away and waits on the second epoch only before it reads the log-rates. The aim is to shorten the helper's idle time at the hand-over by overlapping the stepper's log evaluation with the helper's table construction. In exchange it adds a second spin-wait, drops the reuse/noop hints in this path (always 0, so no-op tables get rebuilt), and adds more kernel instantiations. It is enabled by default whenever the lean path is active.

Result: no change. 17560 billion (median of 6 runs) (+0.7%).

```diff
diff --git a/include/literate_hip.h b/include/literate_hip.h
--- a/include/literate_hip.h
+++ b/include/literate_hip.h
@@ -283,6 +283,7 @@
 int lr_mcmc_p4_resident(const lr_engine* e, int32_t out[4] );
 int lr_mcmc_p4_pipe(const lr_engine* e, int32_t out[4] );
 int lr_mcmc_p4_draws(const lr_engine* e, int32_t* out );
+int lr_mcmc_p4_hand(const lr_engine* e, int32_t* out );
 int lr_mcmc_destroy(lr_engine* e);
 
 #ifdef __cplusplus
diff --git a/literate_amd/_hip.py b/literate_amd/_hip.py
--- a/literate_amd/_hip.py
+++ b/literate_amd/_hip.py
@@ -151,6 +151,7 @@
     "lr_mcmc_p4_resident": (c_i32, [c_vp, C.POINTER(c_i32)]),
     "lr_mcmc_p4_pipe": (c_i32, [c_vp, C.POINTER(c_i32)]),
     "lr_mcmc_p4_draws": (c_i32, [c_vp, C.POINTER(c_i32)]),
+    "lr_mcmc_p4_hand": (c_i32, [c_vp, C.POINTER(c_i32)]),
     "lr_mcmc_status": (c_i32, [c_vp, C.POINTER(c_i32), c_vp]),
     "lr_mcmc_warnings": (c_i32, [c_vp, C.POINTER(c_i32), c_vp]),
     "lr_mcmc_destroy": (c_i32, [c_vp]),
diff --git a/literate_amd/csrc/lr_engine.h b/literate_amd/csrc/lr_engine.h
--- a/literate_amd/csrc/lr_engine.h
+++ b/literate_amd/csrc/lr_engine.h
@@ -38,6 +38,7 @@
     bool p4_resident;
     bool p4_pipe;
     bool p4_lean;
+    bool p4_hand;
     bool packed_scan;
     bool streaming;
     hipEvent_t fork;
@@ -84,6 +85,11 @@
     return lr_p4_pipe_choice(e) && !(env && atoi(env) == 0);
 }
 
+static inline bool lr_p4_hand_choice(const lr_engine* e) {
+    const char* env = getenv("LR_P4_EARLY_HAND");
+    return lr_p4_lean_choice(e) && !(env && atoi(env) == 0);
+}
+
 static inline int lr_spec_mode(const lr_engine* e) {
     if (e->lay.spec_chains_per_team != 1) return 0;
     if (e->lay.team_blocks > 1) return 1;
diff --git a/literate_amd/csrc/lr_mcmc.hip b/literate_amd/csrc/lr_mcmc.hip
--- a/literate_amd/csrc/lr_mcmc.hip
+++ b/literate_amd/csrc/lr_mcmc.hip
@@ -180,7 +180,8 @@
 
 typedef __attribute__((address_space(3))) double lr_lds_f64;
 typedef __attribute__((address_space(3))) int lr_lds_i32;
-template <int PB, int ES, bool PRE = false, int SAMPLER = -1, bool HAND = false, int CFG = LR_P4_CFG_GENERIC, bool LEAN = false>
+template <int PB, int ES, bool PRE = false, int SAMPLER = -1, bool HAND = false, int CFG = LR_P4_CFG_GENERIC, bool LEAN = false,
+          bool EARLY = false>
 __device__ __forceinline__ void lr_persist_step_body(const __attribute__((address_space(3))) lr_step_args* a3, int c, int lane,
                                                      __attribute__((address_space(3))) lr_seg_scratch* scratch3,
                                                      lr_lds_f64* st_f64, lr_lds_i32* st_i32, double lik, lr_lds_f64* table3,
@@ -198,7 +199,7 @@
     else if (PRE) {
         lr_rj_draws pre;
         lr_draws_load(draws, pre, lane);
-        lr_chain_step_core<true, PB, HAND, CFG, LEAN>(st, a, 0, c, lane, (lr_seg_scratch*)scratch3, lik, reinterpret_cast<double2*>((double*)table3),
+        lr_chain_step_core<true, PB, HAND, CFG, LEAN, EARLY>(st, a, 0, c, lane, (lr_seg_scratch*)scratch3, lik, reinterpret_cast<double2*>((double*)table3),
                                            table_es, br_lds, br_lds + LR_H_WIDE, &pre, hand, hand_epoch);
     } else
         lr_chain_step_core<true, PB>(st, a, 0, c, lane, (lr_seg_scratch*)scratch3, lik, reinterpret_cast<double2*>((double*)table3),
@@ -238,7 +239,7 @@
     lr_persist_step_body<PB, ES>(a3, c, lane, scratch3, st_f64, st_i32, lik, table3, br3);
 }
 
-template <int PB, int ES, int NW, int SAMPLER, bool HELP, int CFG = LR_P4_CFG_GENERIC, int TAG = 0, bool LEAN = false>
+template <int PB, int ES, int NW, int SAMPLER, bool HELP, int CFG = LR_P4_CFG_GENERIC, int TAG = 0, bool LEAN = false, bool EARLY = false>
 __device__ __attribute__((noinline)) void lr_persist4_steppers(const __attribute__((address_space(3))) lr_step_args* a3, int c0,
                                                                int n_chains, int wave, int lane,
                                                                __attribute__((address_space(3))) lr_seg_scratch* scratch3,
@@ -259,7 +260,7 @@
                 double lik = 0.0;
 #pragma unroll
                 for (int w2 = 2; w2 < (ES == 2  ? 3 : NW); ++w2) lik += red[(ph * NW + w2) * 2 + wave];
-                lr_persist_step_body<PB, ES, ES == 2  && SAMPLER == 0, SAMPLER, HELP, CFG, LEAN>(
+                lr_persist_step_body<PB, ES, ES == 2  && SAMPLER == 0, SAMPLER, HELP, CFG, LEAN, EARLY>(
                     a3, c, lane, scratch3, st_f64 + (2 * ph + wave) * (LR_STATE_ROWS * LR_ROW),
                     st_i32 + (2 * ph + wave) * (LR_ISTATE_ROWS * LR_ROW), lik, tab + ph * tab_doubles + wave, br3,
                     draws + (2 * ph + wave), HELP ? hands + wave : nullptr, (int)((2 * iter + ph + 1) & 0x3fffffff));
@@ -434,7 +435,7 @@
 #define LR_P4_PIPE 1
 #endif
 template <int H, bool GENERAL, bool PARAM ,
-          bool HELP = false, int CFG = LR_P4_CFG_GENERIC, int NR = 0, int PIPE = 0, bool LEAN = false>
+          bool HELP = false, int CFG = LR_P4_CFG_GENERIC, int NR = 0, int PIPE = 0, bool LEAN = false, bool EARLY = false>
 __global__ __launch_bounds__(LR_P4_THREADS, LR_P4_THREADS / 256) void lr_persist4_kernel(const lr_step_args* __restrict__ ap ,
                                                                        lr_packed_lineages pk, long long n8,
                                                                        lr_p4_shares sh, long long n_iters, char* carry_all) {
@@ -443,6 +444,7 @@
     static_assert(NR == 0 || HELP, "resident groups come with the helper waves");
     static_assert(PIPE == 0 || (PIPE == 1 && NR > 0), "the one-block form is one of the resident trips");
     static_assert(!LEAN || PIPE > 0, "the lean draw duty comes with the one-block form");
+    static_assert(!EARLY || LEAN, "the two-stage hand-over comes with the lean draw duty");
     const lr_step_args& a = *ap;
     LR_PSTAMP(0);
     constexpr int NW = LR_P4_THREADS / LR_WAVE;
@@ -502,7 +504,25 @@
         if (CFG == LR_P4_CFG_BDI) __builtin_assume((unsigned int)model < 2u);
         if (CFG == LR_P4_CFG_KEIDING) model = LR_MODEL_KEIDING;
         constexpr bool fixed = CFG != LR_P4_CFG_GENERIC;
-        const double constP = lr_build_tables_segments<(H <= 264 ? lr_bins_per_lane(H) : 1), 2>(
+        double constP;
+        if constexpr (EARLY) {
+            constexpr int P = lr_bins_per_lane(H);
+            auto between = [&](const lr_seg_cache*) {
+#ifdef LR_DIAG
+                const unsigned long long dh1 = wall_clock64();
+#endif
+                while (__hip_atomic_load(&hand->epoch2, __ATOMIC_RELAXED, __HIP_MEMORY_SCOPE_WORKGROUP) != epoch) __builtin_amdgcn_s_sleep(1);
+                asm volatile("" ::: "memory");
+#ifdef LR_DIAG
+                if (lane == 0 && blockIdx.x < 64) atomicAdd(&lr_diag_step[16384 + (blockIdx.x * 16 + wave) * 4 + 3], wall_clock64() - dh1);
+#endif
+            };
+            constP = lr_build_tables_segments_fast<P, 2, true>(sc, eL, eM, hand->KL, hand->KM, br_lds[0], br_lds[1], model, a_lds.cfg.n_bins,
+                                                               fixed ? H : a_lds.H, reinterpret_cast<double2*>(tabd), lane, LR_TAB_UNIT,
+                                                               fixed ? LR_P4_FRAC_BIRTH : a_lds.cfg.frac_birth,
+                                                               fixed ? LR_P4_FRAC_DEATH : a_lds.cfg.frac_death, ES, nullptr, between);
+        } else
+        constP = lr_build_tables_segments<(H <= 264 ? lr_bins_per_lane(H) : 1), 2>(
             sc, eL, eM, hand->KL, hand->KM, br_lds[0], br_lds[1], model, a_lds.cfg.n_bins, a_lds.n_cls, fixed ? H : a_lds.H,
             reinterpret_cast<double2*>(tabd), lane, LR_TAB_UNIT, fixed ? LR_P4_FRAC_BIRTH : a_lds.cfg.frac_birth,
             fixed ? LR_P4_FRAC_DEATH : a_lds.cfg.frac_death, ES, nullptr);
@@ -512,6 +532,7 @@
     };
     if (tid == 0) arrived = 0;
     if (tid < 2) hands[tid].epoch = 0;
+    if (EARLY && tid < 2) hands[tid].epoch2 = 0;
     for (int i = tid; i < 2 * NW * 2; i += LR_P4_THREADS) (&red[0][0][0])[i] = 0.0;
     int scans_done = 0;
     constexpr int NA = NS + (HELP ? 2 : 0);
@@ -622,7 +643,7 @@
             }
         }
     } else if (!scanner)
-        lr_persist4_steppers<(H <= 264 ? lr_bins_per_lane(H) : 0), ES, NW, PARAM ? 1 : 0, HELP, CFG, NR + 64 * PIPE, LEAN>(
+        lr_persist4_steppers<(H <= 264 ? lr_bins_per_lane(H) : 0), ES, NW, PARAM ? 1 : 0, HELP, CFG, NR + 64 * PIPE, LEAN, EARLY>(
             (const __attribute__((address_space(3))) lr_step_args*)&a_lds, c0, C, wave, lane,
             (__attribute__((address_space(3))) lr_seg_scratch*)&scratch[wave], (lr_lds_f64*)&st_f64[0][0], (lr_lds_i32*)&st_i32[0][0],
             (lr_lds_f64*)&red[0][0][0], (lr_lds_f64*)reinterpret_cast<double*>(tab[0]), 2 * LR_UNIT_PLANES * H,
@@ -829,6 +850,7 @@
     e->p4_resident = lr_p4_resident_choice(e);
     e->p4_pipe = lr_p4_pipe_choice(e);
     e->p4_lean = lr_p4_lean_choice(e);
+    e->p4_hand = lr_p4_hand_choice(e);
     e->streaming = false;
     e->packed_scan = plan.packed_scan;
     e->fork = nullptr;
@@ -1151,6 +1173,12 @@
         if (general && param) hipLaunchKernelGGL((lr_persist4_kernel<HH, true, true>), g4, b4, 0, stream, ap, pk, e->n8, e->p4, (long long)n, p4_carry);   \
         else if (general) hipLaunchKernelGGL((lr_persist4_kernel<HH, true, false>), g4, b4, 0, stream, ap, pk, e->n8, e->p4, (long long)n, p4_carry);      \
         else if (param) hipLaunchKernelGGL((lr_persist4_kernel<HH, false, true>), g4, b4, 0, stream, ap, pk, e->n8, e->p4, (long long)n, p4_carry);        \
+        else if (LR_P4_NR > 0 && LR_P4_PIPE > 0 && e->p4_help && e->p4_resident && e->p4_pipe && e->p4_lean && e->p4_hand && e->p4_cfg == LR_P4_CFG_BDI)    \
+            hipLaunchKernelGGL((lr_persist4_kernel<(HH <= 264 ? HH : 264), false, false, true, LR_P4_CFG_BDI, LR_P4_NR, LR_P4_PIPE, true, true>), g4, b4, 0, stream, ap, pk, e->n8, e->p4, (long long)n, p4_carry); \
+        else if (LR_P4_NR > 0 && LR_P4_PIPE > 0 && e->p4_help && e->p4_resident && e->p4_pipe && e->p4_lean && e->p4_hand && e->p4_cfg == LR_P4_CFG_KEIDING)                               \
+            hipLaunchKernelGGL((lr_persist4_kernel<(HH <= 264 ? HH : 264), false, false, true, LR_P4_CFG_KEIDING, LR_P4_NR, LR_P4_PIPE, true, true>), g4, b4, 0, stream, ap, pk, e->n8, e->p4, (long long)n, p4_carry); \
+        else if (LR_P4_NR > 0 && LR_P4_PIPE > 0 && e->p4_help && e->p4_resident && e->p4_pipe && e->p4_lean && e->p4_hand)                                                                 \
+            hipLaunchKernelGGL((lr_persist4_kernel<(HH <= 264 ? HH : 264), false, false, true, LR_P4_CFG_GENERIC, LR_P4_NR, LR_P4_PIPE, true, true>), g4, b4, 0, stream, ap, pk, e->n8, e->p4, (long long)n, p4_carry); \
         else if (LR_P4_NR > 0 && LR_P4_PIPE > 0 && e->p4_help && e->p4_resident && e->p4_pipe && e->p4_lean && e->p4_cfg == LR_P4_CFG_BDI)    \
             hipLaunchKernelGGL((lr_persist4_kernel<(HH <= 264 ? HH : 264), false, false, true, LR_P4_CFG_BDI, LR_P4_NR, LR_P4_PIPE, true>), g4, b4, 0, stream, ap, pk, e->n8, e->p4, (long long)n, p4_carry); \
         else if (LR_P4_NR > 0 && LR_P4_PIPE > 0 && e->p4_help && e->p4_resident && e->p4_pipe && e->p4_lean && e->p4_cfg == LR_P4_CFG_KEIDING)                                   \
@@ -1294,6 +1322,12 @@
     return LR_OK;
 }
 
+extern "C" int lr_mcmc_p4_hand(const lr_engine* e, int32_t* out) {
+    if (!e || !out) return LR_ERR_NULL;
+    *out = (e->plan.family == 2 && e->p4_help && e->p4_resident && e->p4_pipe && e->p4_lean && e->p4_hand && LR_P4_NR > 0 && LR_P4_PIPE > 0) ? 1 : 0;
+    return LR_OK;
+}
+
 extern "C" int lr_mcmc_p4_draws(const lr_engine* e, int32_t* out) {
     if (!e || !out) return LR_ERR_NULL;
     *out = (e->plan.family == 2 && e->p4_help && e->p4_resident && e->p4_pipe && e->p4_lean && LR_P4_NR > 0 && LR_P4_PIPE > 0) ? 1 : 0;
diff --git a/literate_amd/csrc/lr_pack.hip b/literate_amd/csrc/lr_pack.hip
--- a/literate_amd/csrc/lr_pack.hip
+++ b/literate_amd/csrc/lr_pack.hip
@@ -156,6 +156,7 @@
     e->p4_resident = lr_p4_resident_choice(e);
     e->p4_pipe = lr_p4_pipe_choice(e);
     e->p4_lean = lr_p4_lean_choice(e);
+    e->p4_hand = lr_p4_hand_choice(e);
     if (e->lay.persistent == 2 && e->p4_help) {
         static const int env_t = lr_env_int("LR_P4_HELP_TRIPS", -1);
         const double t = ((double)e->n8 + 512.0) / 896.0;
diff --git a/literate_amd/csrc/lr_step.h b/literate_amd/csrc/lr_step.h
--- a/literate_amd/csrc/lr_step.h
+++ b/literate_amd/csrc/lr_step.h
@@ -174,13 +174,17 @@
     *packL = pl, *packM = pm;
 }
 
-template <int P, int CS = 2>
+struct lr_tables_no_wait {
+    __device__ __forceinline__ void operator()(const lr_seg_cache*) const {}
+};
+
+template <int P, int CS = 2, bool LATE_LOGS = false, class BETWEEN = lr_tables_no_wait>
 __device__ __forceinline__ double lr_build_tables_segments_fast(const lr_seg_scratch* sc, int eL, int eM, int KL,
                                                                 int KM, const double* __restrict__ br_length,
                                                                 const double* __restrict__ log_br, int model,
                                                                 int n_bins, int H, double2* __restrict__ tab,
                                                                 int lane, int unit, double fs0, double fe0, int es,
-                                                                lr_seg_cache* sg = nullptr) {
+                                                                lr_seg_cache* sg = nullptr, BETWEEN between = BETWEEN()) {
     double* tabd = reinterpret_cast<double*>(tab);
     auto put_S = [&](int j, double v, double R) { lr_put_S<CS>(tabd, unit, es, j, v, R, fs0); };
     auto put_E = [&](int j, double v, double R) { lr_put_E<CS>(tabd, unit, es, j, v, R, fe0); };
@@ -211,7 +215,7 @@
 #pragma unroll
     for (int p = 0; p < P; ++p) {
         const double lam = sc->rate[0][segL[p]], mu = sc->rate[1][segM[p]];
-        const double llam = sc->lograte[0][segL[p]], lmu = sc->lograte[1][segM[p]];
+        const double llam = LATE_LOGS ? 0.0 : sc->lograte[0][segL[p]], lmu = LATE_LOGS ? 0.0 : sc->lograte[1][segM[p]];
         logB[p] = 0.0, logD[p] = 0.0, R[p] = 0.0;
         if (b0 + p < n_bins) {
             if (model >= 2) {
@@ -229,6 +233,21 @@
     double totR;
     double cum = lr_wave_exclusive_scan(sumR, lane, &totR);
     LR_SSTAMP(12);
+    if constexpr (LATE_LOGS) {
+        between(sg);
+#pragma unroll
+        for (int p = 0; p < P; ++p) {
+            const double llam = sc->lograte[0][segL[p]], lmu = sc->lograte[1][segM[p]];
+            if (b0 + p < n_bins) {
+                if (model >= 2) {
+                    logB[p] = llam, logD[p] = lmu;
+                } else if (k_b[p] > 0.0) {
+                    logB[p] = (model == 0) ? lk_b[p] + llam : llam;
+                    logD[p] = lmu + lk_b[p];
+                }
+            }
+        }
+    }
 #pragma unroll
     for (int p = 0; p < P; ++p) {
         const int b = b0 + p;
@@ -574,18 +593,19 @@
     int reuse;
     int noop;
     int out_idx, base_idx;
-    int pad_;
+    int epoch2;
     double par[8];
 };
 
 template <bool LDS_CONSTS = false, int PB = 0, int CS = 2, bool PAIR_PLANES = true, bool HAND = false, int CFG = LR_P4_CFG_GENERIC,
-          bool LEAN = false>
+          bool LEAN = false, bool EARLY = false>
 __device__ __forceinline__ void lr_propose_rj(const lr_step_args& a, int c, int lane, lr_seg_scratch* scratch_p,
                                               uint64_t it, lr_rj_state& s, lr_rj_prop& p, double2* table,
                                               int table_es, const lr_rj_draws* pre = nullptr,
                                               const double* br_lds = nullptr, const double* logbr_lds = nullptr,
                                               const double* base_col = nullptr, int col_doubles = 0, double base_const = 0.0,
                                               lr_table_hand* hand = nullptr, int hand_epoch = 0) {
+    static_assert(!EARLY || HAND, "the two-stage hand-over is one of the helper-wave form");
     static_assert(CS == 2 || (PB > 0 && !PAIR_PLANES), "a column of its own: one-pass builder, no pair planes");
     static_assert(!HAND || PB > 0, "a helper wave runs the one-pass builder");
     static_assert(CFG == LR_P4_CFG_GENERIC || HAND, "a configuration word comes with the helper waves");
@@ -696,6 +716,28 @@
 
     LR_SSTAMP(3);
     double logpL, logpM, log_u_next;
+    if constexpr (EARLY) {
+        const double Mhi = lr_half_lo(pM);
+        const bool hi = lane >= 32;
+        const int j = lane & 31;
+        const bool valid = hi ? (j < PKM) : (j < PKL);
+        const bool free63 = PKM < LR_KMAX;
+        double x = valid ? (hi ? Mhi : pL) : 1.0;
+        if (lane == LR_WAVE - 1 && free63) x = u_next;
+        scratch.rate[hi][j] = x;
+        if (lane <= LR_KMAX) scratch.edge[0][lane] = peL, scratch.edge[1][lane] = peM;
+        if (lane == 0) hand->KL = PKL, hand->KM = PKM, hand->reuse = 0, hand->noop = 0;
+        LR_WAVE_LDS_ORDER();
+        if (lane == 0) __hip_atomic_store(&hand->epoch, hand_epoch, __ATOMIC_RELAXED, __HIP_MEMORY_SCOPE_WORKGROUP);
+        asm volatile("" : "+v"(x) :: "memory");
+        const double lx = lr_log(x);
+        log_u_next = free63 ? lr_bcast(lx, LR_WAVE - 1) : lr_log(u_next);
+        scratch.lograte[hi][j] = lx;
+        logpL = lx;
+        logpM = lr_half_hi(lx);
+        LR_WAVE_LDS_ORDER();
+        if (lane == 0) __hip_atomic_store(&hand->epoch2, hand_epoch, __ATOMIC_RELAXED, __HIP_MEMORY_SCOPE_WORKGROUP);
+    } else
     lr_stage_segments(&scratch, pL, pM, peL, peM, PKL, PKM, lane, &logpL, &logpM, u_next, &log_u_next);
     if (pre && !LEAN) log_u_next = pre->log_u;
 
@@ -704,7 +746,7 @@
     if ((pre && s.sg_valid) || base_col) edges_same = PKL == KL && PKM == KM && __ballot(lane <= LR_KMAX && (peL != eL || peM != eM)) == 0ull;
     if (pre && s.sg_valid) sg.reuse = edges_same;
     const bool same_table = base_col && edges_same && (move_kind == 1 || move_kind == 3 || move_kind == 5);
-    if (HAND) {
+    if (HAND && !EARLY) {
         if (lane == 0) hand->KL = PKL, hand->KM = PKM, hand->reuse = sg.reuse ? 1 : 0, hand->noop = same_table ? 1 : 0;
         LR_WAVE_LDS_ORDER();
         if (lane == 0) __hip_atomic_store(&hand->epoch, hand_epoch, __ATOMIC_RELAXED, __HIP_MEMORY_SCOPE_WORKGROUP);
@@ -756,7 +798,7 @@
     p.gibbs = gibbs, p.invalid = invalid, p.move = move_kind;
 }
 
-template <bool LDS_CONSTS = false, int PB = 0, bool HAND = false, int CFG = LR_P4_CFG_GENERIC, bool LEAN = false>
+template <bool LDS_CONSTS = false, int PB = 0, bool HAND = false, int CFG = LR_P4_CFG_GENERIC, bool LEAN = false, bool EARLY = false>
 __device__ __forceinline__ void lr_chain_step_core(lr_chain_regs& st, const lr_step_args& a, int mode, int c, int lane,
                                                    lr_seg_scratch* scratch_p, double lik_sum, double2* table,
                                                    int table_es = 2, const double* br_lds = nullptr,
@@ -814,7 +856,7 @@
     const int KL = s.KL, KM = s.KM;
 
     lr_rj_prop p;
-    if (HAND) lr_propose_rj<LDS_CONSTS, (PB > 0 ? PB : 1), 2, true, HAND, CFG, LEAN>(a, c, lane, scratch_p, it, s, p, table, table_es, pre, br_lds, logbr_lds, nullptr, 0, 0.0, hand, hand_epoch);
+    if (HAND) lr_propose_rj<LDS_CONSTS, (PB > 0 ? PB : 1), 2, true, HAND, CFG, LEAN, EARLY>(a, c, lane, scratch_p, it, s, p, table, table_es, pre, br_lds, logbr_lds, nullptr, 0, 0.0, hand, hand_epoch);
     else lr_propose_rj<LDS_CONSTS, PB>(a, c, lane, scratch_p, it, s, p, table, table_es, pre, br_lds, logbr_lds);
 
     st.pL = s.L, st.pM = s.M, st.ptL = s.tL, st.ptM = s.tM, st.peL = s.eL, st.peM = s.eM;
diff --git a/literate_amd/engine.py b/literate_amd/engine.py
--- a/literate_amd/engine.py
+++ b/literate_amd/engine.py
@@ -235,6 +235,11 @@
         _hip.check(self.lib.lr_mcmc_p4_draws(self.handle, C.byref(w)), "lr_mcmc_p4_draws")
         return "lean" if w.value else "full"
 
+    def p4_hand(self):
+        w = C.c_int32(0)
+        _hip.check(self.lib.lr_mcmc_p4_hand(self.handle, C.byref(w)), "lr_mcmc_p4_hand")
+        return "early" if w.value else "late"
+
     def timed_steps(self, n):
         ms = C.c_float(0.0)
         _hip.check(self._launch(self.lib.lr_mcmc_time_steps, self.handle, int(n), C.byref(ms)), "lr_mcmc_time_steps")
diff --git a/scratch/diag_p4_waves.py b/scratch/diag_p4_waves.py
--- a/scratch/diag_p4_waves.py
+++ b/scratch/diag_p4_waves.py
@@ -23,4 +23,5 @@
     help_ = eng.kernel_name().endswith("true>")
     role = "step" if w < 2 else ("help" if help_ and w < 4 else "scan")
     print("  w%-2d %s  %.2f / %.2f%s" % (w, role, d[:, w, 0].mean(), d[:, w, 1].mean(),
-                                       "   (of the work: %.2f waiting for the hand-over)" % d[:, w, 2].mean() if role == "help" else ""))
+                                       "   (of the work: %.2f waiting for the hand-over, %.2f for its second stage)"
+                                       % (d[:, w, 2].mean(), d[:, w, 3].mean()) if role == "help" else ""))
```
